# TUMFTM/global_racetrajectory_optimization

Hardware: AMD Instinct MI355X
Metric: min-curv QP solves/sec, N=2000 waypoints, batch=1024 per GPU (higher is better)
Workload: dtype f64

## Files before the change

### __graft_entry__.py

```python
import os
import subprocess
import sys
import tempfile

ROOT = os.path.dirname(os.path.abspath(__file__))
if ROOT not in sys.path:
    sys.path.insert(0, ROOT)


def build() -> None:
    env = dict(os.environ)
    env.setdefault("HIPCC", "/opt/rocm/bin/hipcc")
    fd, asm = tempfile.mkstemp(prefix="mcq_kernels_gfx950_", suffix=".s")
    os.close(fd)
    env["ASM_OUT"] = asm
    subprocess.run([os.path.join(ROOT, "global_racetrajectory_optimization_amd", "csrc", "build.sh")], check=True, env=env)
    build_variants()
    subprocess.run(["make", "-s", "-C", os.path.join(ROOT, "oracle"), "all"], check=True)
    r = subprocess.run([sys.executable, os.path.join(ROOT, "scripts", "check_csr.py"), asm], env=env)
    try:
        os.unlink(asm)
    except OSError:
        pass
    if r.returncode != 0:
        ver = subprocess.run([env["HIPCC"], "--version"], capture_output=True, text=True).stdout
        if "7.2." in ver:
            raise RuntimeError("scripts/check_csr.py found a device function that clobbers a callee-saved SGPR (see its output)")
        print("WARNING: scripts/check_csr.py reported offenders with an untested hipcc version -- not failing the build", file=sys.stderr)
    import global_racetrajectory_optimization_amd
    from global_racetrajectory_optimization_amd import engine
    lib = engine.load_library()
    for sym in engine.EXPORTED_SYMBOLS:
        assert hasattr(lib, sym), sym


VARIANTS = {"ulp": (["-DMCQ_PERTURB_ULP=1"], {}), "ipra": ([], {"IPRA": "1"}), "nocontract": (["-ffp-contract=off"], {}),
            "nof32": (["-DMCQ_IPM_F32=0"], {})}


def variant_path(name):
    return os.path.join(ROOT, "global_racetrajectory_optimization_amd", "csrc", "variants", "libmcq_%s.so" % name)


def build_variants() -> None:
    os.makedirs(os.path.dirname(variant_path("x")), exist_ok=True)
    procs = []
    for name, (flags, extra) in VARIANTS.items():
        env = dict(os.environ)
        env.setdefault("HIPCC", "/opt/rocm/bin/hipcc")
        env.pop("ASM_OUT", None)
        env.update(extra)
        env["OUT"] = variant_path(name)
        procs.append((name, subprocess.Popen([os.path.join(ROOT, "global_racetrajectory_optimization_amd", "csrc", "build.sh")] + flags, env=env)))
    for name, p in procs:
        if p.wait() != 0:
            raise RuntimeError("build of the arithmetic variant '%s' failed" % name)


def smoke() -> None:
    import numpy as np
    from global_racetrajectory_optimization_amd import engine
    from oracle import tph_ref

    g = np.load(os.path.join(ROOT, "tests", "golden", "rounded_rectangle.npz"))
    ref, nv, sc = g["reftrack"], g["normvec"], g["scaling"]
    eng = engine.Engine(0)
    al, curv, st, info = eng.solve_batch([dict(reftrack=ref, normvec=nv, scaling=sc, kappa_bound=0.12, w_veh=3.4)])
    assert st[0] == 0, "engine status %d" % st[0]
    path_cl = np.vstack((ref[:, :2], ref[0, :2]))
    _, _, A, nv_d = tph_ref.calc_splines(path_cl)
    a_ref, err_ref = tph_ref.opt_min_curv(ref, nv_d, A, 0.12, 3.4)
    d = float(np.max(np.abs(al[0] - a_ref)))
    assert d < 1e-6, "alpha differs from the oracle by %.3e m" % d
    assert abs(curv[0] - err_ref) < 1e-9
    assert float(np.max(np.abs(al[0] - g["alpha"]))) < 1e-6
    al_gi, _, st_gi, info_gi = eng.solve_batch([dict(reftrack=ref, normvec=nv, scaling=sc, kappa_bound=0.12, w_veh=3.4)], algorithm=engine.ALG_GI)
    d_gi = float(np.max(np.abs(al_gi[0] - a_ref)))
    assert st_gi[0] == 0 and info_gi[0]["gi_iters"] > 0 and d_gi < 1e-6, "Goldfarb-Idnani path: status %d, alpha differs by %.3e m" % (st_gi[0], d_gi)
    al_sp, _, st_sp, _ = eng.solve_batch([dict(reftrack=ref, normvec=nv, scaling=None, kappa_bound=1.0, w_veh=3.4)],
                                         objective=engine.OBJ_SHORTEST_PATH)
    d_sp = float(np.max(np.abs(al_sp[0] - tph_ref.opt_shortest_path(ref, nv, 3.4))))
    assert st_sp[0] == 0 and d_sp < 1e-6, "shortest path: status %d, alpha differs by %.3e m" % (st_sp[0], d_sp)
    iq = eng.iqp_batch([dict(reftrack=ref, normvectors=nv, scaling=sc)], 0.12, 3.4, 3.0, iters_min=3, curv_error_allowed=0.01)
    d_iqp = float(np.max(np.abs(iq["alpha"][0] - g["iqp_alpha"]))) if iq["alpha"][0].shape == g["iqp_alpha"].shape else float("inf")
    assert iq["status"][0] == 0 and d_iqp < 1e-6, "iqp: status %d, alpha differs by %.3e m" % (iq["status"][0], d_iqp)
    print("smoke ok: N=%d, max|alpha_gpu - alpha_oracle| = %.2e m (Goldfarb-Idnani path %.2e m in %d steps, shortest path %.2e m, iqp end state "
          "%.2e m), curv_error_max = %.6f, info = %s" % (ref.shape[0], d, d_gi, info_gi[0]["gi_iters"], d_sp, d_iqp, curv[0], info[0]))
    eng.close()


if __name__ == "__main__":
    build()
    if len(sys.argv) > 1 and sys.argv[1] == "smoke":
        smoke()
```

### global_racetrajectory_optimization_amd/csrc/mcq_kernels.hip

```cpp
#include "mcq_kernels.h"

#include <math.h>



#define MCQ_NT 256
#define MCQ_NW (MCQ_NT / 64)
typedef double d2 __attribute__((vector_size(16)));
typedef __attribute__((address_space(1))) d2 gd2;

#define SM_RED 0
#define SM_S (SM_RED + 64)
#define SPK 1920
#define SM_OVL (SM_S + SPK)
#define OVL_SIZE 7464
#define SM_KV (SM_OVL + OVL_SIZE)
#define SM_KI (SM_KV + 3 * MCQ_KMAX)
#define SM_TOTAL (SM_KI + (3 * MCQ_KMAX + 2 + 1) / 2 + 1)
static_assert(sizeof(double) * SM_TOTAL <= 80 * 1024, "two workgroups of the solver kernel per CU");

size_t mcq_solve_lds_bytes() { return sizeof(double) * SM_TOTAL; }

__shared__ double g_sm[SM_TOTAL];

#ifndef MCQ_IPM_GM_MIN
#define MCQ_IPM_GM_MIN 0.995
#endif
#ifndef MCQ_IPM_GM_C
#define MCQ_IPM_GM_C 10.0
#endif
#ifndef MCQ_TAPIA_RATIO
#define MCQ_TAPIA_RATIO 0.7
#endif
#ifndef MCQ_TAPIA_SHRINK
#define MCQ_TAPIA_SHRINK 0.7
#endif
#ifndef MCQ_WARM_ROUNDS
#define MCQ_WARM_ROUNDS 12
#endif
#define MCQ_AS_WINDOW 8

__device__ __forceinline__ int cyc1(int i, int n)
{
    i = i < 0 ? i + n : i;
    return i >= n ? i - n : i;
}

__device__ __forceinline__ int cyc(int i, int n)
{
    i %= n;
    return i < 0 ? i + n : i;
}

__device__ __forceinline__ int sdiff(int a, int b, int n)
{
    int d = cyc(a - b, n);
    return d > n / 2 ? d - n : d;
}

__device__ __forceinline__ double wave_sum(double v)
{
    for (int m = 32; m >= 1; m >>= 1) v += __shfl_xor(v, m);
    return v;
}
__device__ __forceinline__ double wave_min(double v)
{
    for (int m = 32; m >= 1; m >>= 1) v = fmin(v, __shfl_xor(v, m));
    return v;
}
__device__ __forceinline__ double wave_max(double v)
{
    for (int m = 32; m >= 1; m >>= 1) v = fmax(v, __shfl_xor(v, m));
    return v;
}

__device__ double block_reduce_(double v, int op, double* red)
{
    const int lane = threadIdx.x & 63, wv = threadIdx.x >> 6;
    v = op == 0 ? wave_sum(v) : (op == 1 ? wave_min(v) : wave_max(v));
    __syncthreads();
    if (lane == 0) red[wv] = v;
    __syncthreads();
    double r = red[0];
    for (int k = 1; k < MCQ_NW; ++k) r = op == 0 ? r + red[k] : (op == 1 ? fmin(r, red[k]) : fmax(r, red[k]));
    return r;
}

__device__ void block_reduce2_(double& a, int opa, double& b, int opb, double* red)
{
    const int lane = threadIdx.x & 63, wv = threadIdx.x >> 6;
    for (int m = 32; m >= 1; m >>= 1) {
        const double oa = __shfl_xor(a, m), ob = __shfl_xor(b, m);
        a = opa == 0 ? a + oa : (opa == 1 ? fmin(a, oa) : fmax(a, oa));
        b = opb == 0 ? b + ob : (opb == 1 ? fmin(b, ob) : fmax(b, ob));
    }
    __syncthreads();
    if (lane == 0) { red[wv] = a; red[MCQ_NW + wv] = b; }
    __syncthreads();
    double ra = red[0], rb = red[MCQ_NW];
    for (int k = 1; k < MCQ_NW; ++k) {
        ra = opa == 0 ? ra + red[k] : (opa == 1 ? fmin(ra, red[k]) : fmax(ra, red[k]));
        rb = opb == 0 ? rb + red[MCQ_NW + k] : (opb == 1 ? fmin(rb, red[MCQ_NW + k]) : fmax(rb, red[MCQ_NW + k]));
    }
    a = ra;
    b = rb;
}

struct McqSet {
    const int* n_list;
    const double* ref;
    const double* nv;
    const double* sc;
    const signed char* warm;
};
__device__ __forceinline__ McqSet mcq_set_of(const McqBatch& B)
{
    McqSet s;
    s.n_list = B.n_list; s.ref = B.ref; s.nv = B.nv; s.sc = B.sc; s.warm = B.warm;
    return s;
}

__device__ __forceinline__ McqWork mcq_work(const McqBatch& B, const McqSet& S, int pb, int& n, double& kb, double& wv)
{
    McqWork w;
    const size_t nm = (size_t)B.nmax;
    n = S.n_list ? S.n_list[pb] : B.n;
    kb = B.kappa_bound_list ? B.kappa_bound_list[pb] : B.kappa_bound;
    wv = B.w_veh_list ? B.w_veh_list[pb] : B.w_veh;
    w.ref = (const gdouble*)(S.ref + (size_t)pb * nm * 4);
    w.nv = S.nv ? (const gdouble*)(S.nv + (size_t)pb * nm * 2) : nullptr;
    w.sc = S.sc ? (const gdouble*)(S.sc + (size_t)pb * nm) : nullptr;
    w.L = (gdouble*)(B.L + (size_t)pb * nm * MCQ_LLD);
    w.vec = (gdouble*)(B.vec + (size_t)pb * nm * MCQ_NVEC);
    w.state = (gschar*)(B.state + (size_t)pb * nm);
    w.Z = (gdouble*)(B.Z + (size_t)pb * MCQ_ZLD(nm));
    w.alpha = B.alpha ? (gdouble*)(B.alpha + (size_t)pb * nm) : nullptr;
    w.curv_err = B.curv_err ? (gdouble*)(B.curv_err + pb) : nullptr;
    w.status = (gint*)(B.status + pb);
    w.info = B.info ? (ginfo*)(B.info + pb) : nullptr;
    return w;
}
__device__ __forceinline__ McqWork mcq_work(const McqBatch& B, int pb, int& n, double& kb, double& wv)
{
    return mcq_work(B, mcq_set_of(B), pb, n, kb, wv);
}

#define VEC(w, nmax, id) ((w).vec + (size_t)(id) * (size_t)(nmax))

template <int N> __device__ __forceinline__ double bcast_row16(double v)
{
    return __builtin_amdgcn_update_dpp(0.0, v, 0x150 + N, 0xf, 0xf, true);
}
#ifndef MCQ_HAVE_FNMA_BCAST_ROW16
template <int N> __device__ __forceinline__ double fnma_bcast_row16(double a, double b, double c)
{
    asm("s_nop 1\n\tv_fmac_f64_dpp %0, %1, -%2 row_newbcast:%3 row_mask:0xf bank_mask:0xf" : "+v"(c) : "v"(a), "v"(b), "n"(N));
    return c;
}
#endif

#ifndef MCQ_IPM_TOL
#define MCQ_IPM_TOL 1e-10
#endif
struct SolveCtx {
    McqDims d;
    McqWork w;
    int nm;
    int direct;
    int max_ipm_iter, max_as_iter, refine_steps;
    double zscale, fscale, wmean, nfree, kbound;
    mutable long long tk[8];
    mutable int refine_rounds, second_attempt, f32_count;
    mutable double last_step;
    mutable const gdouble* sp_sig;
    mutable const gschar* sp_mk;
    mutable const gdouble* kkt_w;
    mutable int kkt_f32;
    mutable int out_iters, out_nk;
    mutable double out_kkt;
    int chain, fix_s, fix_e;
    double psi_s, psi_e;
};
typedef __attribute__((address_space(3))) SolveCtx LCtx;
__shared__ SolveCtx g_ctx;
#define G_CTX (*(const LCtx*)&g_ctx)
#define TICK() ((long long)wall_clock64())
#include "mcq_kkt.inc"
#include "mcq_tri.inc"

#ifndef MCQ_ENTRY_BATCH
#define MCQ_ENTRY_BATCH 1
#endif
#define EB_E (MCQ_ENTRY_BATCH ? 8 : 1)
#define EB_FOR for (int eb0_ = tid; eb0_ < n; eb0_ += EB_E * MCQ_NT)
#define EB_EACH _Pragma("unroll") for (int u = 0; u < EB_E; ++u)
#define EB_INDEX                                                                                                       \
    int idx[EB_E];                                                                                                     \
    bool ok[EB_E];                                                                                                     \
    EB_EACH {                                                                                                          \
        ok[u] = eb0_ + u * MCQ_NT < n;                                                                                 \
        idx[u] = ok[u] ? eb0_ + u * MCQ_NT : eb0_;                                                                     \
    }

__device__ __noinline__ int assemble_problem(const LCtx& c, double wveh, gdouble* nv_out, gdouble* sc_out)
{
    double* red = g_sm + SM_RED;
    const int tid = threadIdx.x;
    McqWork w;
    w.ref = c.w.ref; w.nv = c.w.nv; w.sc = c.w.sc; w.L = c.w.L; w.vec = c.w.vec; w.state = c.w.state; w.Z = c.w.Z;
    w.alpha = c.w.alpha; w.curv_err = c.w.curv_err; w.status = c.w.status; w.info = c.w.info;
    const int nm = c.nm, n = c.d.n;
    gdouble* LO = VEC(w, nm, V_LO);
    gdouble* HI = VEC(w, nm, V_HI);
    gdouble* S = VEC(w, nm, V_SC);
    gdouble* XP = VEC(w, nm, V_XP);
    gdouble* YP = VEC(w, nm, V_YP);
    gdouble* CP = VEC(w, nm, V_CP);
    gdouble* KRF = VEC(w, nm, V_KREF);
    gdouble* XPP = VEC(w, nm, V_XPP);
    gdouble* YPP = VEC(w, nm, V_YPP);

    double flag_bad = 0.0, flag_inf = 0.0;
    if (n < 3) flag_bad = 1.0;
    gdouble* NX = VEC(w, nm, V_NX);
    gdouble* NY = VEC(w, nm, V_NY);
    const bool derive = w.nv == nullptr;
    const bool chain = c.chain != 0;
    if (chain && (n > MCQ_CHAIN_MAXN || derive || !(isfinite(c.psi_s) && isfinite(c.psi_e)))) flag_bad = 1.0;
    EB_FOR {
        EB_INDEX
        double rx[EB_E], ry[EB_E], rwr[EB_E], rwl[EB_E], rnx[EB_E], rny[EB_E], rs[EB_E], x1[EB_E], y1[EB_E], x2[EB_E], y2[EB_E];
        EB_EACH {
            const int i = idx[u];
            rx[u] = w.ref[4 * i]; ry[u] = w.ref[4 * i + 1]; rwr[u] = w.ref[4 * i + 2]; rwl[u] = w.ref[4 * i + 3];
            rnx[u] = derive ? 0.0 : w.nv[2 * i]; rny[u] = derive ? 1.0 : w.nv[2 * i + 1];
            rs[u] = w.sc ? w.sc[i] : 1.0;
            x1[u] = y1[u] = x2[u] = y2[u] = 0.0;
            if (derive) {
                const int i1 = i + 1 >= n ? i + 1 - n : i + 1, i2 = i1 + 1 >= n ? i1 + 1 - n : i1 + 1;
                x1[u] = w.ref[4 * i1]; y1[u] = w.ref[4 * i1 + 1]; x2[u] = w.ref[4 * i2]; y2[u] = w.ref[4 * i2 + 1];
            }
        }
        EB_EACH {
            if (!ok[u]) continue;
            const int i = idx[u];
            const double x = rx[u], y = ry[u], wr = rwr[u], wl = rwl[u];
            const double nx = rnx[u], ny = rny[u];
            double s = rs[u];
            if (chain && i >= n - 2) s = 1.0;
            if (derive) {
                const double l0 = hypot(x1[u] - x, y1[u] - y);
                const double l1 = hypot(x2[u] - x1[u], y2[u] - y1[u]);
                s = l0 / l1;
            } else {
                NX[i] = nx;
                NY[i] = ny;
            }
            if (!(isfinite(x) && isfinite(y) && isfinite(wr) && isfinite(wl) && isfinite(nx) && isfinite(ny) && isfinite(s)
                  && s > 0.0))
                flag_bad = 1.0;
            double lo = -(wl - 0.5 * wveh), hi = wr - 0.5 * wveh;
            if ((c.fix_s && i == 0) || (c.fix_e && i == n - 1)) { lo = -MCQ_FIX_HALF_WIDTH; hi = MCQ_FIX_HALF_WIDTH; }
            if (hi < lo) flag_inf = 1.0;
            LO[i] = lo;
            HI[i] = hi;
            S[i] = s;
        }
    }
    flag_bad = block_reduce_(flag_bad, 2, red);
    flag_inf = block_reduce_(flag_inf, 2, red);
    const int st = flag_bad > 0.0 ? MCQ_BAD_INPUT : (flag_inf > 0.0 ? MCQ_INFEASIBLE : MCQ_OK);
    if (tid == 0) {
        *w.status = st;
        if (w.curv_err) *w.curv_err = 0.0;
        if (w.info) {
            mcq_info z;
            z.ipm_iters = z.as_iters = z.n_active_box = z.n_active_kappa = 0;
            z.kappa_max = 0.0;
            z.kkt_res = 0.0;
            z.refine_rounds = z.second_attempt = z.f32_factorisations = z.gi_iters = 0;
            for (int q = 0; q < 8; ++q) z.ticks[q] = 0;
            *(mcq_info*)w.info = z;
        }
    }
    if (st != MCQ_OK) {
        if (w.alpha) for (int i = tid; i < n; i += MCQ_NT) w.alpha[i] = 0.0;
        return st;
    }
    __syncthreads();

    tri_prepare(c);
    gdouble* RX = VEC(w, nm, V_SK);
    gdouble* RY = VEC(w, nm, V_EDA);
    EB_FOR {
        EB_INDEX
        double sm1[EB_E], xp_[EB_E], yp_[EB_E], x0[EB_E], y0[EB_E], xm_[EB_E], ym_[EB_E];
        EB_EACH {
            const int m = idx[u], mp = cyc1(m + 1, n), mm = cyc1(m - 1, n);
            sm1[u] = S[mm];
            xp_[u] = w.ref[4 * mp]; yp_[u] = w.ref[4 * mp + 1]; x0[u] = w.ref[4 * m]; y0[u] = w.ref[4 * m + 1]; xm_[u] = w.ref[4 * mm]; ym_[u] = w.ref[4 * mm + 1];
        }
        EB_EACH if (ok[u]) {
            RX[idx[u]] = 3.0 * (sm1[u] * (xp_[u] - x0[u]) - (x0[u] - xm_[u]));
            RY[idx[u]] = 3.0 * (sm1[u] * (yp_[u] - y0[u]) - (y0[u] - ym_[u]));
        }
    }
    double hsx = 0.0, hsy = 0.0, hex = 0.0, hey = 0.0;
    if (chain) {
        hsx = MCQ_HEADING_SCALE * cos(c.psi_s + 0.5 * M_PI);
        hsy = MCQ_HEADING_SCALE * sin(c.psi_s + 0.5 * M_PI);
        hex = MCQ_HEADING_SCALE * cos(c.psi_e + 0.5 * M_PI);
        hey = MCQ_HEADING_SCALE * sin(c.psi_e + 0.5 * M_PI);
        __syncthreads();
    }
    if (chain && tid == 0) {
        RX[0] = 3.0 * ((w.ref[4] - w.ref[0]) - hsx);
        RY[0] = 3.0 * ((w.ref[5] - w.ref[1]) - hsy);
        RX[n - 1] = 3.0 * (hex - (w.ref[4 * (n - 1)] - w.ref[4 * (n - 2)]));
        RY[n - 1] = 3.0 * (hey - (w.ref[4 * (n - 1) + 1] - w.ref[4 * (n - 2) + 1]));
    }
    tri_solve_T(c, RX, XPP);
    tri_solve_T(c, RY, YPP);
    EB_FOR {
        EB_INDEX
        double a[EB_E], b[EB_E];
        EB_EACH { a[u] = XPP[idx[u]]; b[u] = YPP[idx[u]]; }
        EB_EACH if (ok[u]) { XPP[idx[u]] = a[u] * 2.0; YPP[idx[u]] = b[u] * 2.0; }
    }
    __syncthreads();

    EB_FOR {
        EB_INDEX
        double si[EB_E], xn_[EB_E], yn_[EB_E], x0[EB_E], y0[EB_E], ax[EB_E], axn[EB_E], ay[EB_E], ayn[EB_E];
        EB_EACH {
            const int i = idx[u], ip = cyc(i + 1, n);
            si[u] = S[i];
            xn_[u] = w.ref[4 * ip]; yn_[u] = w.ref[4 * ip + 1]; x0[u] = w.ref[4 * i]; y0[u] = w.ref[4 * i + 1];
            ax[u] = XPP[i]; axn[u] = XPP[ip]; ay[u] = YPP[i]; ayn[u] = YPP[ip];
        }
        EB_EACH {
            if (!ok[u]) continue;
            const int i = idx[u];
            const double s2 = si[u] * si[u];
            const double xp = (xn_[u] - x0[u]) - (ax[u] + 0.5 * s2 * axn[u]) / 3.0;
            const double yp = (yn_[u] - y0[u]) - (ay[u] + 0.5 * s2 * ayn[u]) / 3.0;
            const double den = pow(xp * xp + yp * yp, 1.5);
            const double cp = den != 0.0 ? 1.0 / den : 0.0;
            XP[i] = xp;
            YP[i] = yp;
            CP[i] = cp;
            KRF[i] = cp * (xp * ay[u] - yp * ax[u]);
            if (derive) {
                const double nrm = sqrt(xp * xp + yp * yp);
                NX[i] = yp / nrm;
                NY[i] = -xp / nrm;
            }
            if (nv_out) {
                nv_out[2 * i] = NX[i];
                nv_out[2 * i + 1] = NY[i];
            }
            if (sc_out) sc_out[i] = si[u];
        }
    }
    if (chain) {
        __syncthreads();
        if (tid == 0) {
            const int i = n - 1;
            const double den = pow(hex * hex + hey * hey, 1.5);
            const double cp = den != 0.0 ? 1.0 / den : 0.0;
            XP[i] = hex;
            YP[i] = hey;
            CP[i] = cp;
            KRF[i] = cp * (hex * YPP[i] - hey * XPP[i]);
        }
    }
    __syncthreads();
    return MCQ_OK;
}

__device__ __forceinline__ void ctx_set_problem(const McqBatch& B, const McqSet& S, int pb, int& n, double& kb, double& wveh)
{
    const McqWork w = mcq_work(B, S, pb, n, kb, wveh);
    __syncthreads();
    if (threadIdx.x == 0) {
        g_ctx.w = w;
        g_ctx.nm = B.nmax;
        g_ctx.d = mcq_dims(n);
        const mcq_ends* e = B.ends ? B.ends + pb : nullptr;
        g_ctx.chain = (e && !e->closed) ? 1 : 0;
        g_ctx.fix_s = g_ctx.chain && e->fix_s;
        g_ctx.fix_e = g_ctx.chain && e->fix_e;
        g_ctx.psi_s = g_ctx.chain ? e->psi_s : 0.0;
        g_ctx.psi_e = g_ctx.chain ? e->psi_e : 0.0;
    }
    __syncthreads();
}

__device__ __forceinline__ void ctx_set_problem(const McqBatch& B, int pb, int& n, double& kb, double& wveh)
{
    ctx_set_problem(B, mcq_set_of(B), pb, n, kb, wveh);
}

__device__ __forceinline__ void ctx_set_solve(const McqBatch& B, double kbound)
{
    if (threadIdx.x == 0) {
        for (int q = 0; q < 8; ++q) g_ctx.tk[q] = 0;
        g_ctx.last_step = 0.0;
        g_ctx.refine_rounds = g_ctx.second_attempt = g_ctx.f32_count = 0;
        g_ctx.direct = B.objective == MCQ_OBJ_SHORTEST_PATH;
        g_ctx.max_ipm_iter = B.max_ipm_iter;
        g_ctx.max_as_iter = B.max_as_iter;
        g_ctx.refine_steps = B.refine_steps;
        g_ctx.kbound = kbound;
        g_ctx.kkt_w = nullptr;
        g_ctx.kkt_f32 = 0;
        g_ctx.sp_sig = nullptr;
        g_ctx.sp_mk = nullptr;
        g_ctx.out_iters = g_ctx.out_nk = 0;
        g_ctx.out_kkt = 0.0;
    }
    __syncthreads();
}

__global__ void __launch_bounds__(MCQ_NT) mcq_assemble_kernel(McqBatch B)
{
    int n;
    double kb, wveh;
    ctx_set_problem(B, blockIdx.x, n, kb, wveh);
    const size_t nm = (size_t)B.nmax;
    (void)assemble_problem(G_CTX, wveh, B.nv_out ? (gdouble*)(B.nv_out + (size_t)blockIdx.x * nm * 2) : nullptr,
                           B.sc_out ? (gdouble*)(B.sc_out + (size_t)blockIdx.x * nm) : nullptr);
}

__global__ void __launch_bounds__(MCQ_NT) mcq_assemble_sp_kernel(McqBatch B)
{
    __shared__ double red[64];
    const int tid = threadIdx.x;
    int n;
    double kb, wveh;
    const McqWork w = mcq_work(B, blockIdx.x, n, kb, wveh);
    const int nm = B.nmax;
    gdouble* LO = VEC(w, nm, V_LO);
    gdouble* HI = VEC(w, nm, V_HI);
    gdouble* NX = VEC(w, nm, V_NX);
    gdouble* NY = VEC(w, nm, V_NY);
    gdouble* F = VEC(w, nm, V_F);
    gdouble* KRF = VEC(w, nm, V_KREF);

    double flag_bad = n < 3 ? 1.0 : 0.0;
    for (int i = tid; i < n; i += MCQ_NT) {
        const double x = w.ref[4 * i], y = w.ref[4 * i + 1], wr = w.ref[4 * i + 2], wl = w.ref[4 * i + 3];
        const double nx = w.nv[2 * i], ny = w.nv[2 * i + 1];
        if (!(isfinite(x) && isfinite(y) && isfinite(wr) && isfinite(wl) && isfinite(nx) && isfinite(ny))) flag_bad = 1.0;
        NX[i] = nx;
        NY[i] = ny;
        LO[i] = -fmax(wl - 0.5 * wveh, 0.001);
        HI[i] = fmax(wr - 0.5 * wveh, 0.001);
        KRF[i] = 0.0;
    }
    flag_bad = block_reduce_(flag_bad, 2, red);
    const int st = flag_bad > 0.0 ? MCQ_BAD_INPUT : MCQ_OK;
    if (tid == 0) {
        *w.status = st;
        if (w.curv_err) *w.curv_err = 0.0;
        if (w.info) {
            mcq_info z;
            z.ipm_iters = z.as_iters = z.n_active_box = z.n_active_kappa = 0;
            z.kappa_max = 0.0;
            z.kkt_res = 0.0;
            z.refine_rounds = z.second_attempt = z.f32_factorisations = z.gi_iters = 0;
            for (int q = 0; q < 8; ++q) z.ticks[q] = 0;
            *(mcq_info*)w.info = z;
        }
    }
    if (st != MCQ_OK) {
        if (w.alpha) for (int i = tid; i < n; i += MCQ_NT) w.alpha[i] = 0.0;
        return;
    }

    gdouble* HD = VEC(w, nm, V_XP);
    gdouble* HU = VEC(w, nm, V_YP);
    for (int i = tid; i < n; i += MCQ_NT) {
        const int ip = i + 1 == n ? 0 : i + 1, im = i == 0 ? n - 1 : i - 1;
        HD[i] = 4.0 * (w.nv[2 * i] * w.nv[2 * i] + w.nv[2 * i + 1] * w.nv[2 * i + 1]);
        HU[i] = -2.0 * (w.nv[2 * i] * w.nv[2 * ip] + w.nv[2 * i + 1] * w.nv[2 * ip + 1]);
        const double px = w.ref[4 * i], py = w.ref[4 * i + 1];
        F[i] = 2.0 * (w.nv[2 * i] * ((px - w.ref[4 * im]) - (w.ref[4 * ip] - px))
                      + w.nv[2 * i + 1] * ((py - w.ref[4 * im + 1]) - (w.ref[4 * ip + 1] - py)));
    }
}


__device__ __noinline__ int factor(const LCtx& c, const gdouble* sig, const gschar* mk, gdouble* fv, bool f32)
{
    if (c.direct) return factor_sp(c, sig, mk);
    c.kkt_f32 = f32 ? 1 : 0;
    if (threadIdx.x == 0) c.f32_count += f32 ? 1 : 0;
    return f32 ? factor_kkt<true>(c, sig, mk, c.kkt_w, fv) : factor_kkt<false>(c, sig, mk, c.kkt_w, fv);
}

__device__ __noinline__ void solve(const LCtx& c, gdouble* v, bool fwd_done)
{
    if (c.direct) { (void)sp_solve(c, v, v); return; }
    if (c.kkt_f32) solve_kkt<true>(c, v, fwd_done);
    else solve_kkt<false>(c, v, fwd_done);
}

__device__ __forceinline__ void apply_Et(const LCtx& c, const gdouble* src, gdouble* dst) { tri_apply_Et(c, src, dst); }

__device__ __noinline__ void gradient(const LCtx& c, const gdouble* x, const gdouble* extra, gdouble* tmp, gdouble* g)
{
    const int n = c.d.n;
    const long long t0 = TICK();
    __syncthreads();
    if (c.direct) {
        const gdouble* HD = VEC(c.w, c.nm, V_SPD);
        const gdouble* HU = VEC(c.w, c.nm, V_SPU);
        const gdouble* F = VEC(c.w, c.nm, V_F);
        for (int i = threadIdx.x; i < n; i += MCQ_NT) {
            const int im = i > 0 ? i - 1 : n - 1, ip = i + 1 < n ? i + 1 : 0;
            g[i] = F[i] + HU[im] * x[im] + HD[i] * x[i] + HU[i] * x[ip];
        }
        __syncthreads();
        if (threadIdx.x == 0) c.tk[2] += TICK() - t0;
        return;
    }
    tri_apply_E(c, x, VEC(c.w, c.nm, V_KREF), MCQ_F_SCALE, tmp);
    if (extra) {
        for (int i = threadIdx.x; i < n; i += MCQ_NT) tmp[i] += extra[i];
        __syncthreads();
    }
    tri_apply_Et(c, tmp, g);
    if (threadIdx.x == 0) c.tk[2] += TICK() - t0;
}

__device__ __forceinline__ int timed_factor(const LCtx& c, const gdouble* sig, const gschar* mk, gdouble* fv = nullptr, bool f32 = false)
{
    const long long t0 = TICK();
    const int r = factor(c, sig, mk, fv, f32);
    if (threadIdx.x == 0) c.tk[0] += TICK() - t0;
    return r;
}
__device__ __forceinline__ void timed_solve(const LCtx& c, gdouble* v, bool fwd_done = false)
{
    const long long t0 = TICK();
    solve(c, v, fwd_done);
    if (threadIdx.x == 0) c.tk[1] += TICK() - t0;
}


__device__ __noinline__ int ipm(const LCtx& c, bool with_kappa)
{
    const int tid = threadIdx.x, n = c.d.n, nm = c.nm;
    double* red = g_sm + SM_RED;
    const gdouble* LO = VEC(c.w, nm, V_LO);
    const gdouble* HI = VEC(c.w, nm, V_HI);
    const gdouble* KR = VEC(c.w, nm, V_KREF);
    gdouble* X = VEC(c.w, nm, V_X);
    gdouble* G = VEC(c.w, nm, V_G);
    gdouble* ZL = VEC(c.w, nm, V_ZL);
    gdouble* ZU = VEC(c.w, nm, V_ZU);
    gdouble* SIG = VEC(c.w, nm, V_SIG);
    gdouble* RHS = VEC(c.w, nm, V_RHS);
    gdouble* DXA = VEC(c.w, nm, V_DXA);
    gdouble* T0 = VEC(c.w, nm, V_T0);
    gdouble* T1 = VEC(c.w, nm, V_T1);
    gdouble* T2 = VEC(c.w, nm, V_T2);
    gdouble* TL = VEC(c.w, nm, V_TL);
    gdouble* TU = VEC(c.w, nm, V_TU);
    gdouble* YL = VEC(c.w, nm, V_YL);
    gdouble* YU = VEC(c.w, nm, V_YU);
    gdouble* SK = VEC(c.w, nm, V_SK);
    gdouble* EDA = VEC(c.w, nm, V_EDA);
    gdouble* Q = VEC(c.w, nm, V_Q);
    gschar* ST = c.w.state;
    const double kb = c.kbound, zscale = c.zscale;
    const double IPM_TOL = 1e-10;
    c.out_iters = 0;

    for (int i = tid; i < n; i += MCQ_NT) {
        const bool fixed = !(HI[i] - LO[i] > 1e-12);
        ST[i] = fixed ? 2 : 0;
        X[i] = 0.5 * (LO[i] + HI[i]);
        ZL[i] = fixed ? 0.0 : zscale;
        ZU[i] = ZL[i];
    }
    __syncthreads();
    if (with_kappa) {
        tri_apply_E(c, X, KR, 1.0, T0);
        const double mu0 = 0.5 * zscale * c.wmean;
        for (int i = tid; i < n; i += MCQ_NT) {
            const double r = T0[i];
            const double tl = fmax(kb + r, 0.1 * kb), tu = fmax(kb - r, 0.1 * kb);
            TL[i] = tl; TU[i] = tu;
            YL[i] = mu0 / tl; YU[i] = mu0 / tu;
        }
        __syncthreads();
    }
    const double npairs = 2.0 * c.nfree + (with_kappa ? 2.0 * n : 0.0);
    const gschar* const no_mask = nullptr;
    const bool any_fixed = c.nfree < (double)n;
    (void)no_mask;
    if (!(npairs > 0.0)) return MCQ_OK;

    bool g_exact = true;
    double mu_first = 0.0, rdm_best = 1e300;
    for (int it = 1; it <= c.max_ipm_iter; ++it) {
        if (with_kappa) {
            for (int i = tid; i < n; i += MCQ_NT) Q[i] = YU[i] - YL[i];
            gradient(c, X, Q, T0, T1);
            gradient(c, X, nullptr, T0, G);
            tri_apply_E(c, X, KR, 1.0, T0);
        }
        double mu, rdm, rhom;
        for (;;) {
            mu = 0.0; rdm = 0.0; rhom = 0.0;
            for (int i = tid; i < n; i += MCQ_NT) {
                if (with_kappa) {
                    mu += TL[i] * YL[i] + TU[i] * YU[i];
                    rhom = fmax(rhom, fmax(fabs(TL[i] - (kb + T0[i])), fabs(TU[i] - (kb - T0[i]))));
                    SK[i] = YL[i] / TL[i] + YU[i] / TU[i];
                }
                if (ST[i] != 0) continue;
                const double sl = X[i] - LO[i], su = HI[i] - X[i];
                mu += sl * ZL[i] + su * ZU[i];
                const double gg = with_kappa ? T1[i] : G[i];
                rdm = fmax(rdm, fabs(gg - ZL[i] + ZU[i]));
                SIG[i] = ZL[i] / sl + ZU[i] / su;
            }
            mu = block_reduce_(mu, 0, red) / npairs;
            rdm = block_reduce_(rdm, 2, red);
            rhom = block_reduce_(rhom, 2, red);
            const bool conv = mu < IPM_TOL * zscale * c.wmean && rdm < IPM_TOL * zscale && rhom <= 1e-9 * kb;
            if (with_kappa && it > 1 && mu < 1e-6 * mu_first && rdm > 10.0 * rdm_best) return MCQ_OK;
            rdm_best = fmin(rdm_best, rdm);
#ifdef IPM_TRACE
            if (tid == 0) printf("ipm%d it %d mu %.3e rdm %.3e rhom %.3e step %.3e\n", (int)with_kappa, it, mu / (zscale * c.wmean), rdm / zscale, rhom / kb, c.last_step);
#endif
            if (conv && (with_kappa || g_exact)) return MCQ_OK;
            if (!conv) break;
            gradient(c, X, nullptr, T0, G);
            g_exact = true;
        }
        c.out_iters = it;
        if (it == 1) mu_first = mu;

        int fs;
        if (with_kappa) {
            for (int i = tid; i < n; i += MCQ_NT) EDA[i] = 1.0 + SK[i];
            __syncthreads();
            c.kkt_w = EDA;
            fs = timed_factor(c, SIG, any_fixed ? ST : nullptr);
            c.kkt_w = nullptr;
            if (fs == MCQ_NOT_PD && mu < 1e-6 * mu_first) return MCQ_OK;
        } else {
            fs = timed_factor(c, SIG, any_fixed ? ST : nullptr);
        }
        if (fs != 0) return fs;

        if (with_kappa) {
            for (int i = tid; i < n; i += MCQ_NT) {
                const double rl = TL[i] - (kb + T0[i]), ru = TU[i] - (kb - T0[i]);
                Q[i] = YL[i] * rl / TL[i] - YU[i] * ru / TU[i];
            }
            __syncthreads();
            apply_Et(c, Q, T2);
            __syncthreads();
            for (int i = tid; i < n; i += MCQ_NT) RHS[i] = ST[i] == 0 ? -G[i] + T2[i] : 0.0;
        } else {
            for (int i = tid; i < n; i += MCQ_NT) RHS[i] = ST[i] == 0 ? -G[i] : 0.0;
        }
        timed_solve(c, RHS);
        if (with_kappa) {
            tri_apply_E(c, RHS, nullptr, 0.0, EDA);
        }
        double ap = 1.0, ad = 1.0;
        for (int i = tid; i < n; i += MCQ_NT) {
            if (with_kappa) {
                const double rl = TL[i] - (kb + T0[i]), ru = TU[i] - (kb - T0[i]);
                const double dtl = EDA[i] - rl, dtu = -EDA[i] - ru;
                const double dyl = -YL[i] - YL[i] * dtl / TL[i], dyu = -YU[i] - YU[i] * dtu / TU[i];
                if (dtl < 0.0) ap = fmin(ap, -TL[i] / dtl);
                if (dtu < 0.0) ap = fmin(ap, -TU[i] / dtu);
                if (dyl < 0.0) ad = fmin(ad, -YL[i] / dyl);
                if (dyu < 0.0) ad = fmin(ad, -YU[i] / dyu);
            }
            if (ST[i] != 0) { DXA[i] = 0.0; continue; }
            const double dx = RHS[i];
            DXA[i] = dx;
            const double sl = X[i] - LO[i], su = HI[i] - X[i];
            const double dzl = -ZL[i] - ZL[i] * dx / sl, dzu = -ZU[i] + ZU[i] * dx / su;
            if (dx < 0.0) ap = fmin(ap, -sl / dx);
            if (dx > 0.0) ap = fmin(ap, su / dx);
            if (dzl < 0.0) ad = fmin(ad, -ZL[i] / dzl);
            if (dzu < 0.0) ad = fmin(ad, -ZU[i] / dzu);
        }
        ap = block_reduce_(ap, 1, red);
        ad = block_reduce_(ad, 1, red);
        double mua = 0.0;
        for (int i = tid; i < n; i += MCQ_NT) {
            if (with_kappa) {
                const double rl = TL[i] - (kb + T0[i]), ru = TU[i] - (kb - T0[i]);
                const double dtl = EDA[i] - rl, dtu = -EDA[i] - ru;
                const double dyl = -YL[i] - YL[i] * dtl / TL[i], dyu = -YU[i] - YU[i] * dtu / TU[i];
                mua += (TL[i] + ap * dtl) * (YL[i] + ad * dyl) + (TU[i] + ap * dtu) * (YU[i] + ad * dyu);
            }
            if (ST[i] != 0) continue;
            const double dx = DXA[i];
            const double sl = X[i] - LO[i], su = HI[i] - X[i];
            const double dzl = -ZL[i] - ZL[i] * dx / sl, dzu = -ZU[i] + ZU[i] * dx / su;
            mua += (sl + ap * dx) * (ZL[i] + ad * dzl) + (su - ap * dx) * (ZU[i] + ad * dzu);
        }
        mua = block_reduce_(mua, 0, red) / npairs;
        const double ratio = mua / mu;
        const double smu = ratio * ratio * ratio * mu;

        if (with_kappa) {
            for (int i = tid; i < n; i += MCQ_NT) {
                const double rl = TL[i] - (kb + T0[i]), ru = TU[i] - (kb - T0[i]);
                const double dtl = EDA[i] - rl, dtu = -EDA[i] - ru;
                const double dyl = -YL[i] - YL[i] * dtl / TL[i], dyu = -YU[i] - YU[i] * dtu / TU[i];
                Q[i] = (smu - dtl * dyl + YL[i] * rl) / TL[i] - (smu - dtu * dyu + YU[i] * ru) / TU[i];
            }
            __syncthreads();
            apply_Et(c, Q, T2);
            __syncthreads();
        }
        for (int i = tid; i < n; i += MCQ_NT) {
            if (ST[i] != 0) { RHS[i] = 0.0; continue; }
            const double dx = DXA[i];
            const double sl = X[i] - LO[i], su = HI[i] - X[i];
            const double dzl = -ZL[i] - ZL[i] * dx / sl, dzu = -ZU[i] + ZU[i] * dx / su;
            RHS[i] = -G[i] + (smu - dx * dzl) / sl - (smu + dx * dzu) / su + (with_kappa ? T2[i] : 0.0);
        }
        timed_solve(c, RHS);
        if (with_kappa) {
            tri_apply_E(c, RHS, nullptr, 0.0, Q);
        }
        double amax = 1.0 / 0.995;
        for (int i = tid; i < n; i += MCQ_NT) {
            if (with_kappa) {
                const double rl = TL[i] - (kb + T0[i]), ru = TU[i] - (kb - T0[i]);
                const double dtla = EDA[i] - rl, dtua = -EDA[i] - ru;
                const double dyla = -YL[i] - YL[i] * dtla / TL[i], dyua = -YU[i] - YU[i] * dtua / TU[i];
                const double dtl = Q[i] - rl, dtu = -Q[i] - ru;
                const double dyl = (-TL[i] * YL[i] + smu - dtla * dyla - YL[i] * dtl) / TL[i];
                const double dyu = (-TU[i] * YU[i] + smu - dtua * dyua - YU[i] * dtu) / TU[i];
                EDA[i] = dyl;
                SK[i] = dyu;
                if (dtl < 0.0) amax = fmin(amax, -TL[i] / dtl);
                if (dtu < 0.0) amax = fmin(amax, -TU[i] / dtu);
                if (dyl < 0.0) amax = fmin(amax, -YL[i] / dyl);
                if (dyu < 0.0) amax = fmin(amax, -YU[i] / dyu);
            }
            if (ST[i] != 0) continue;
            const double dx = RHS[i], da = DXA[i];
            const double sl = X[i] - LO[i], su = HI[i] - X[i];
            const double dzla = -ZL[i] - ZL[i] * da / sl, dzua = -ZU[i] + ZU[i] * da / su;
            const double dzl = (-sl * ZL[i] + smu - da * dzla - ZL[i] * dx) / sl;
            const double dzu = (-su * ZU[i] + smu + da * dzua + ZU[i] * dx) / su;
            T1[i] = dzl;
            T2[i] = dzu;
            if (dx < 0.0) amax = fmin(amax, -sl / dx);
            if (dx > 0.0) amax = fmin(amax, su / dx);
            if (dzl < 0.0) amax = fmin(amax, -ZL[i] / dzl);
            if (dzu < 0.0) amax = fmin(amax, -ZU[i] / dzu);
        }
        amax = block_reduce_(amax, 1, red);
        const double a = fmin(1.0, 0.995 * amax);
        c.last_step = a;
        for (int i = tid; i < n; i += MCQ_NT) {
            if (with_kappa) {
                const double rl = TL[i] - (kb + T0[i]), ru = TU[i] - (kb - T0[i]);
                TL[i] += a * (Q[i] - rl);
                TU[i] += a * (-Q[i] - ru);
                YL[i] += a * EDA[i];
                YU[i] += a * SK[i];
            }
            if (ST[i] != 0) continue;
            if (!with_kappa) {
                const double dxa = DXA[i], dx = RHS[i];
                const double sl = X[i] - LO[i], su = HI[i] - X[i];
                const double dzla = -ZL[i] - ZL[i] * dxa / sl, dzua = -ZU[i] + ZU[i] * dxa / su;
                const double rc = -G[i] + (smu - dxa * dzla) / sl - (smu + dxa * dzua) / su;
                G[i] += a * (rc - SIG[i] * dx);
            }
            {
                const double sl = X[i] - LO[i], su = HI[i] - X[i];
                const double rsl = (sl + a * RHS[i]) * ZL[i], rzl = (ZL[i] + a * T1[i]) * sl;
                const double rsu = (su - a * RHS[i]) * ZU[i], rzu = (ZU[i] + a * T2[i]) * su;
                const bool al = rsl < MCQ_TAPIA_RATIO * rzl && sl + a * RHS[i] < MCQ_TAPIA_SHRINK * sl, au = rsu < MCQ_TAPIA_RATIO * rzu && su - a * RHS[i] < MCQ_TAPIA_SHRINK * su;
                VEC(c.w, nm, V_T3)[i] = al ? -1.0 : (au ? 1.0 : 0.0);
            }
            X[i] += a * RHS[i];
            ZL[i] += a * T1[i];
            ZU[i] += a * T2[i];
        }
        g_exact = false;
        __syncthreads();
    }
    return with_kappa ? MCQ_KAPPA_INFEASIBLE : MCQ_ITER_CAP;
}

#define IPB_E 8
#define IPB_H 4
#ifndef MCQ_IPB_RESIDENT
#define MCQ_IPB_RESIDENT 1
#endif
#ifndef MCQ_IPB_DEFER
#define MCQ_IPB_DEFER MCQ_IPB_RESIDENT
#endif
#ifndef MCQ_IPB_NOCOPY
#define MCQ_IPB_NOCOPY MCQ_IPB_RESIDENT
#endif
#if MCQ_IPB_DEFER && !MCQ_IPB_RESIDENT
#error "MCQ_IPB_DEFER needs MCQ_IPB_RESIDENT"
#endif
#ifndef MCQ_IPB_FOLD_P1
#define MCQ_IPB_FOLD_P1 1
#endif
__device__ __noinline__ int ipm_box(const LCtx& c, double tol, bool resume)
{
#define IPB_SETUP                                                                                                      \
    const int tid = threadIdx.x, n = c.d.n, nm = c.nm;                                                                 \
    double* red = g_sm + SM_RED;                                                                                       \
    const gdouble* LO = VEC(c.w, nm, V_LO);                                                                            \
    const gdouble* HI = VEC(c.w, nm, V_HI);                                                                            \
    gdouble* X = VEC(c.w, nm, V_X);                                                                                    \
    gdouble* G = VEC(c.w, nm, V_G);                                                                                    \
    gdouble* ZL = VEC(c.w, nm, V_ZL);                                                                                  \
    gdouble* ZU = VEC(c.w, nm, V_ZU);                                                                                  \
    gdouble* SIG = VEC(c.w, nm, V_SIG);                                                                                \
    gdouble* RHS = VEC(c.w, nm, V_RHS);                                                                                \
    gdouble* DXA = VEC(c.w, nm, V_DXA);                                                                                \
    gschar* ST = c.w.state;                                                                                            \
    gdouble* IND = VEC(c.w, nm, V_T3);                                                                                 \
    (void)IND; (void)red; (void)LO; (void)HI; (void)X; (void)G; (void)ZL; (void)ZU; (void)SIG; (void)RHS; (void)DXA; (void)ST;    \
    int idx[IPB_E];                                                                                                    \
    bool ok[IPB_E];                                                                                                    \
    _Pragma("unroll") for (int u = 0; u < IPB_E; ++u) {                                                                \
        ok[u] = tid + u * MCQ_NT < n;                                                                                  \
        idx[u] = ok[u] ? tid + u * MCQ_NT : 0;           \
    }
#define IPB_HALF(h)                                                                                                    \
    int idx[IPB_H];                                                                                                    \
    bool ok[IPB_H];                                                                                                    \
    _Pragma("unroll") for (int u = 0; u < IPB_H; ++u) {                                                                \
        ok[u] = tid + ((h) * IPB_H + u) * MCQ_NT < n;                                                                  \
        idx[u] = ok[u] ? tid + ((h) * IPB_H + u) * MCQ_NT : 0;                                                         \
    }
#define IPB_PTRS                                                                                                       \
    const int tid = threadIdx.x, n = c.d.n, nm = c.nm;                                                                 \
    double* red = g_sm + SM_RED;                                                                                       \
    const gdouble* LO = VEC(c.w, nm, V_LO);                                                                            \
    const gdouble* HI = VEC(c.w, nm, V_HI);                                                                            \
    gdouble* X = VEC(c.w, nm, V_X);                                                                                    \
    gdouble* G = VEC(c.w, nm, V_G);                                                                                    \
    gdouble* ZL = VEC(c.w, nm, V_ZL);                                                                                  \
    gdouble* ZU = VEC(c.w, nm, V_ZU);                                                                                  \
    gdouble* SIG = VEC(c.w, nm, V_SIG);                                                                                \
    gdouble* RHS = VEC(c.w, nm, V_RHS);                                                                                \
    gdouble* DXA = VEC(c.w, nm, V_DXA);                                                                                \
    gschar* ST = c.w.state;                                                                                            \
    gdouble* IND = VEC(c.w, nm, V_T3);                                                                                 \
    (void)IND; (void)red; (void)LO; (void)HI; (void)X; (void)G; (void)ZL; (void)ZU; (void)SIG; (void)RHS; (void)DXA; (void)ST;
#if MCQ_IPB_NOCOPY
#define IPB_CORR DXA
#define IPB_PRED RHS
#else
#define IPB_CORR RHS
#define IPB_PRED DXA
#endif
    const double zscale = c.zscale;
    const double IPM_TOL = tol;
    c.out_iters = 0;
    {
    IPB_SETUP
#if MCQ_ENTRY_BATCH
    double lo[IPB_E], hi[IPB_E];
#pragma unroll
    for (int u = 0; u < IPB_E; ++u) { lo[u] = LO[idx[u]]; hi[u] = HI[idx[u]]; }
#define IPB_LO(u, i) lo[u]
#define IPB_HI(u, i) hi[u]
#else
#define IPB_LO(u, i) LO[i]
#define IPB_HI(u, i) HI[i]
#endif
#pragma unroll
    for (int u = 0; u < IPB_E; ++u) {
        if (!ok[u]) continue;
        const int i = idx[u];
        const bool fixed = !(IPB_HI(u, i) - IPB_LO(u, i) > 1e-12);
        ST[i] = fixed ? 2 : 0;
        if (!resume) {
            X[i] = 0.5 * (IPB_LO(u, i) + IPB_HI(u, i));
            ZL[i] = fixed ? 0.0 : zscale;
            ZU[i] = ZL[i];
        }
    }
#undef IPB_LO
#undef IPB_HI
    }
    __syncthreads();
    if (resume) gradient(c, VEC(c.w, c.nm, V_X), nullptr, VEC(c.w, c.nm, V_T0), VEC(c.w, c.nm, V_G));
    const double npairs = 2.0 * c.nfree;
    const bool any_fixed = c.nfree < (double)c.d.n;
    if (!(npairs > 0.0)) return MCQ_OK;
#if MCQ_IPB_RESIDENT
    double rx[IPB_E], rl[IPB_E], ru[IPB_E], rg[IPB_E];
    {
        IPB_SETUP
#pragma unroll
        for (int u = 0; u < IPB_E; ++u) { const int i = idx[u]; rx[u] = X[i]; rl[u] = ZL[i]; ru[u] = ZU[i]; rg[u] = G[i]; }
    }
#define IPB_RELOAD_G { _Pragma("unroll") for (int u = 0; u < IPB_E; ++u) rg[u] = G[tid + u * MCQ_NT < n ? tid + u * MCQ_NT : 0]; }
#else
#define IPB_RELOAD_G
#endif
#if MCQ_IPB_DEFER
#define IPB_STORE_X { _Pragma("unroll") for (int u = 0; u < IPB_E; ++u) if (tid + u * MCQ_NT < n) X[tid + u * MCQ_NT] = rx[u]; }
#define IPB_RETURN(v) { rc = (v); goto ipb_flush; }
    unsigned tapia = 0;
    int rc;
#else
#define IPB_STORE_X
#define IPB_RETURN(v) return (v);
#endif

    bool g_exact = true;
    double mu_prev = 1e300;
    int stalled = 0;
#ifndef MCQ_IPM_F32
#define MCQ_IPM_F32 1
#endif
#ifndef MCQ_IPM_F32_RD
#define MCQ_IPM_F32_RD 1e-5
#endif
    bool f32 = MCQ_IPM_F32 && !resume;
#ifndef MCQ_IPM_TRUST_FP64_CARRY
#define MCQ_IPM_TRUST_FP64_CARRY 1
#endif
    bool g_f32 = false;
#if MCQ_IPB_FOLD_P1
    bool folded = false;
    double mu_fold = 0.0, rdm_fold = 0.0;
#endif
    for (int it = 1; it <= c.max_ipm_iter; ++it) {
        double mu;
        for (;;) {
            IPB_PTRS
            double rdm = 0.0;
            mu = 0.0;
#if MCQ_IPB_FOLD_P1
            if (folded) { mu = mu_fold; rdm = rdm_fold; folded = false; }
            else
#endif
            {
#pragma unroll
            for (int h = 0; h < IPB_E / IPB_H; ++h) {
                IPB_HALF(h)
                double x[IPB_H], lo[IPB_H], hi[IPB_H], zl[IPB_H], zu[IPB_H], g[IPB_H];
                int st[IPB_H];
#pragma unroll
                for (int u = 0; u < IPB_H; ++u) {
                    const int i = idx[u];
#if MCQ_IPB_RESIDENT
                    st[u] = ST[i]; lo[u] = LO[i]; hi[u] = HI[i];
                    x[u] = rx[h * IPB_H + u]; zl[u] = rl[h * IPB_H + u]; zu[u] = ru[h * IPB_H + u]; g[u] = rg[h * IPB_H + u];
#else
                    st[u] = ST[i]; x[u] = X[i]; lo[u] = LO[i]; hi[u] = HI[i]; zl[u] = ZL[i]; zu[u] = ZU[i]; g[u] = G[i];
#endif
                }
#pragma unroll
                for (int u = 0; u < IPB_H; ++u) {
                    if (!ok[u]) continue;
                    const int i = idx[u];
                    if (st[u] != 0) { RHS[i] = 0.0; continue; }
                    const double sl = x[u] - lo[u], su = hi[u] - x[u];
                    mu += sl * zl[u] + su * zu[u];
                    rdm = fmax(rdm, fabs(g[u] - zl[u] + zu[u]));
                    SIG[i] = zl[u] / sl + zu[u] / su;
                    RHS[i] = -g[u];
                }
            }
            block_reduce2_(mu, 0, rdm, 2, red);
            mu /= npairs;
            }
            const bool conv = mu < IPM_TOL * zscale * c.wmean && rdm < IPM_TOL * zscale;
#ifdef IPM_TRACE
            if (threadIdx.x == 0) printf("ipmb it %d mu %.3e rdm %.3e exact %d resume %d [%a %a]\n", it, mu / (zscale * c.wmean), rdm / zscale, (int)g_exact, (int)resume, mu, rdm);
#endif
            if (f32 && it > 1 && rdm < MCQ_IPM_F32_RD * zscale) {
                f32 = false;
                if (!g_exact) {
                    IPB_STORE_X
                    gradient(c, X, nullptr, VEC(c.w, nm, V_T0), G);
                    IPB_RELOAD_G
                    g_exact = true;
                    g_f32 = false;
                    continue;
                }
            }
            if (conv && (g_exact || (MCQ_IPM_TRUST_FP64_CARRY && !resume && !g_f32))) IPB_RETURN(MCQ_OK)
            if (!conv) break;
            IPB_STORE_X
            gradient(c, X, nullptr, VEC(c.w, nm, V_T0), G);
            IPB_RELOAD_G
            g_exact = true;
            g_f32 = false;
        }
        c.out_iters = it;
        if (resume) {
            stalled = mu > 0.9 * mu_prev ? stalled + 1 : 0;
            mu_prev = mu;
            if (stalled >= 3) IPB_RETURN(MCQ_OK)
        }

        const int fs = timed_factor(c, VEC(c.w, c.nm, V_SIG), any_fixed ? c.w.state : nullptr,
                                    VEC(c.w, c.nm, V_RHS), f32);
        if (fs != 0) IPB_RETURN((resume && fs == MCQ_NOT_PD) ? MCQ_OK : fs)
        timed_solve(c, VEC(c.w, c.nm, V_RHS), true);

        double smu;
        {
            IPB_SETUP
            double dxa[IPB_E], sl[IPB_E], su[IPB_E], zl[IPB_E], zu[IPB_E], g[IPB_E];
            bool act[IPB_E];
#pragma unroll
            for (int u = 0; u < IPB_E; ++u) {
                const int i = idx[u];
                act[u] = ok[u] && ST[i] == 0;
#if MCQ_IPB_RESIDENT
                const double x = rx[u];
                dxa[u] = RHS[i]; sl[u] = x - LO[i]; su[u] = HI[i] - x; zl[u] = rl[u]; zu[u] = ru[u]; g[u] = rg[u];
#else
                const double x = X[i];
                dxa[u] = RHS[i]; sl[u] = x - LO[i]; su[u] = HI[i] - x; zl[u] = ZL[i]; zu[u] = ZU[i]; g[u] = G[i];
#endif
            }
            double ap = 1.0, ad = 1.0;
#pragma unroll
            for (int u = 0; u < IPB_E; ++u) {
                if (!ok[u]) continue;
#if MCQ_IPB_NOCOPY
                if (!act[u]) continue;
                const double dx = dxa[u];
#else
                if (!act[u]) { DXA[idx[u]] = 0.0; continue; }
                const double dx = dxa[u];
                DXA[idx[u]] = dx;
#endif
                const double dzla = -zl[u] - zl[u] * dx / sl[u];
                const double dzua = -zu[u] + zu[u] * dx / su[u];
                if (dx < 0.0) ap = fmin(ap, -sl[u] / dx);
                if (dx > 0.0) ap = fmin(ap, su[u] / dx);
                if (dzla < 0.0) ad = fmin(ad, -zl[u] / dzla);
                if (dzua < 0.0) ad = fmin(ad, -zu[u] / dzua);
            }
            block_reduce2_(ap, 1, ad, 1, red);
            double mua = 0.0;
#pragma unroll
            for (int u = 0; u < IPB_E; ++u) {
                if (!act[u]) continue;
                const double dzla = -zl[u] - zl[u] * dxa[u] / sl[u];
                const double dzua = -zu[u] + zu[u] * dxa[u] / su[u];
                mua += (sl[u] + ap * dxa[u]) * (zl[u] + ad * dzla) + (su[u] - ap * dxa[u]) * (zu[u] + ad * dzua);
            }
            mua = block_reduce_(mua, 0, red) / npairs;
            const double ratio = mua / mu;
            smu = ratio * ratio * ratio * mu;
#pragma unroll
            for (int u = 0; u < IPB_E; ++u) {
                if (!ok[u]) continue;
                const double dzla = -zl[u] - zl[u] * dxa[u] / sl[u];
                const double dzua = -zu[u] + zu[u] * dxa[u] / su[u];
                IPB_CORR[idx[u]] = act[u] ? -g[u] + (smu - dxa[u] * dzla) / sl[u] - (smu + dxa[u] * dzua) / su[u] : 0.0;
            }
        }
        timed_solve(c, VEC(c.w, c.nm, MCQ_IPB_NOCOPY ? V_DXA : V_RHS));

        {
            IPB_SETUP
#ifdef MCQ_IPM_FIXED_STEP
            const double gm = 0.995;
#else
            const double gm = fmin(fmax(MCQ_IPM_GM_MIN, 1.0 - MCQ_IPM_GM_C * mu / (zscale * c.wmean)), 1.0 - 1e-9);
#endif
            double amax = 1.0 / gm;
            double dx[IPB_E], da[IPB_E], x[IPB_E], lo[IPB_E], hi[IPB_E], zl[IPB_E], zu[IPB_E], g[IPB_E], sg[IPB_E];
            bool act[IPB_E];
#pragma unroll
            for (int u = 0; u < IPB_E; ++u) {
                const int i = idx[u];
                act[u] = ok[u] && ST[i] == 0;
                dx[u] = IPB_CORR[i]; da[u] = IPB_PRED[i]; lo[u] = LO[i]; hi[u] = HI[i]; sg[u] = SIG[i];
#if MCQ_IPB_RESIDENT
                x[u] = rx[u]; zl[u] = rl[u]; zu[u] = ru[u]; g[u] = rg[u];
#else
                x[u] = X[i]; zl[u] = ZL[i]; zu[u] = ZU[i]; g[u] = G[i];
#endif
            }
#define IPB_STEP3(u)                                                                                                          \
                const double sl = x[u] - lo[u], su = hi[u] - x[u];                                                              \
                const double dzla = -zl[u] - zl[u] * da[u] / sl, dzua = -zu[u] + zu[u] * da[u] / su;                             \
                const double dzl = (-sl * zl[u] + smu - da[u] * dzla - zl[u] * dx[u]) / sl;                                     \
                const double dzu = (-su * zu[u] + smu + da[u] * dzua + zu[u] * dx[u]) / su;
#pragma unroll
            for (int u = 0; u < IPB_E; ++u) {
                if (!act[u]) continue;
                IPB_STEP3(u)
                if (dx[u] < 0.0) amax = fmin(amax, -sl / dx[u]);
                if (dx[u] > 0.0) amax = fmin(amax, su / dx[u]);
                if (dzl < 0.0) amax = fmin(amax, -zl[u] / dzl);
                if (dzu < 0.0) amax = fmin(amax, -zu[u] / dzu);
            }
            amax = block_reduce_(amax, 1, red);
            const double a = fmin(1.0, gm * amax);
            c.last_step = a;
#if MCQ_IPB_DEFER
            unsigned t3[IPB_E];
#pragma unroll
            for (int u = 0; u < IPB_E; ++u) t3[u] = 0;
#endif
#if MCQ_IPB_FOLD_P1
            double mu_n = 0.0, rdm_n = 0.0;
#endif
#pragma unroll
            for (int u = 0; u < IPB_E; ++u) {
#if MCQ_IPB_FOLD_P1
                if (ok[u] && !act[u]) RHS[idx[u]] = 0.0;
#endif
                if (!act[u]) continue;
                const int i = idx[u];
                IPB_STEP3(u)
                const double rc = -g[u] + (smu - da[u] * dzla) / sl - (smu + da[u] * dzua) / su;
                const double hdx = rc - sg[u] * dx[u];
                const double gn = g[u] + a * hdx, xn = x[u] + a * dx[u], zln = zl[u] + a * dzl, zun = zu[u] + a * dzu;
#if MCQ_IPB_RESIDENT
                rg[u] = gn; rx[u] = xn; rl[u] = zln; ru[u] = zun;
#endif
#if !MCQ_IPB_DEFER
                G[i] = gn;
                X[i] = xn;
                ZL[i] = zln;
                ZU[i] = zun;
#endif
                const double rsl = (sl + a * dx[u]) * zl[u], rzl = (zl[u] + a * dzl) * sl;
                const double rsu = (su - a * dx[u]) * zu[u], rzu = (zu[u] + a * dzu) * su;
                const bool al = rsl < MCQ_TAPIA_RATIO * rzl && sl + a * dx[u] < MCQ_TAPIA_SHRINK * sl, au = rsu < MCQ_TAPIA_RATIO * rzu && su - a * dx[u] < MCQ_TAPIA_SHRINK * su;
#if MCQ_IPB_DEFER
                t3[u] = al ? 1u : (au ? 3u : 2u);
                (void)i;
#else
                IND[i] = al ? -1.0 : (au ? 1.0 : 0.0);
#endif
#if MCQ_IPB_FOLD_P1
                {
                    const double sl = xn - lo[u], su = hi[u] - xn;
                    mu_n += sl * zln + su * zun;
                    rdm_n = fmax(rdm_n, fabs(gn - zln + zun));
                    SIG[idx[u]] = zln / sl + zun / su;
                    RHS[idx[u]] = -gn;
                }
#endif
            }
#if MCQ_IPB_FOLD_P1
            block_reduce2_(mu_n, 0, rdm_n, 2, red);
            mu_fold = mu_n / npairs;
            rdm_fold = rdm_n;
            folded = true;
#endif
#if MCQ_IPB_DEFER
            tapia = 0;
#pragma unroll
            for (int u = 0; u < IPB_E; ++u) tapia |= t3[u] << (2 * u);
#endif
#undef IPB_STEP3
        }
        g_exact = false;
        g_f32 |= f32;
#if !MCQ_IPB_FOLD_P1
        __syncthreads();
#endif
    }
#if MCQ_IPB_DEFER
    rc = MCQ_ITER_CAP;
ipb_flush:
    {
        IPB_SETUP
#pragma unroll
        for (int u = 0; u < IPB_E; ++u) {
            if (!ok[u]) continue;
            const int i = idx[u];
            X[i] = rx[u]; ZL[i] = rl[u]; ZU[i] = ru[u]; G[i] = rg[u];
            const unsigned t = (tapia >> (2 * u)) & 3u;
            if (t != 0) IND[i] = (double)((int)t - 2);
        }
    }
    __syncthreads();
    return rc;
#else
    return MCQ_ITER_CAP;
#endif
#undef IPB_SETUP
#undef IPB_RELOAD_G
#undef IPB_STORE_X
#undef IPB_RETURN
#undef IPB_CORR
#undef IPB_PRED
}

struct KappaMem {
    double* kmu;
    double* krh;
    double* mul;
    int* ki;
    int* piv;
    gdouble* sg;
    int cap, ld;
    bool in_lds;
};
__device__ __forceinline__ KappaMem kappa_mem_lds(const LCtx& c)
{
    KappaMem k;
    k.kmu = g_sm + SM_KV;
    k.krh = g_sm + SM_KV + MCQ_KMAX;
    k.mul = g_sm + SM_KV + 2 * MCQ_KMAX;
    k.ki = (int*)(g_sm + SM_KI);
    k.piv = (int*)(g_sm + SM_KI) + 1 + 2 * MCQ_KMAX;
    k.sg = c.w.Z + c.nm;
    k.cap = MCQ_KMAX;
    k.ld = MCQ_KMAX;
    k.in_lds = true;
    return k;
}
__device__ __forceinline__ KappaMem kappa_mem_slot(double* slot)
{
    KappaMem k;
    k.sg = (gdouble*)slot;
    double* v = slot + (size_t)MCQ_KBIG * MCQ_KBIG;
    k.kmu = v;
    k.krh = v + MCQ_KBIG;
    k.mul = v + 2 * MCQ_KBIG;
    k.ki = (int*)(v + 3 * MCQ_KBIG);
    k.piv = k.ki + 2 + 2 * MCQ_KBIG;
    k.cap = MCQ_KBIG;
    k.ld = MCQ_KBIG;
    k.in_lds = false;
    return k;
}

template <typename PA>
__device__ __forceinline__ void kappa_lu_eliminate(PA A, int lda, int nk, double* mul, int* piv)
{
    const int tid = threadIdx.x;
    double* red = g_sm + SM_RED;
    for (int cidx = 0; cidx < nk; ++cidx) {
        double best = -1.0;
        int brow = cidx;
        for (int r = cidx + tid; r < nk; r += MCQ_NT) {
            const double v = fabs(A[(size_t)r * lda + cidx]);
            if (v > best) { best = v; brow = r; }
        }
        const double bmax = block_reduce_(best, 2, red);
        double cand = (best == bmax && best >= 0.0) ? (double)brow : 1e300;
        cand = block_reduce_(cand, 1, red);
        const int pr = cand < 1e299 ? (int)cand : cidx;
        if (tid == 0) piv[cidx] = pr;
        if (pr != cidx)
            for (int cc = tid; cc < nk; cc += MCQ_NT) {
                const double t = A[(size_t)cidx * lda + cc];
                A[(size_t)cidx * lda + cc] = A[(size_t)pr * lda + cc];
                A[(size_t)pr * lda + cc] = t;
            }
        __syncthreads();
        const double pv = A[(size_t)cidx * lda + cidx];
        for (int r = cidx + 1 + tid; r < nk; r += MCQ_NT) mul[r] = pv != 0.0 ? A[(size_t)r * lda + cidx] / pv : 0.0;
        __syncthreads();
        const int rem = nk - cidx - 1;
        for (int e = tid; e < rem * rem; e += MCQ_NT) {
            const int r = cidx + 1 + e / rem, cc = cidx + 1 + e % rem;
            A[(size_t)r * lda + cc] -= mul[r] * A[(size_t)cidx * lda + cc];
        }
        __syncthreads();
        for (int r = cidx + 1 + tid; r < nk; r += MCQ_NT) A[(size_t)r * lda + cidx] = mul[r];
        __syncthreads();
    }
}

__device__ void kappa_lu_factor(const KappaMem& K, int nk)
{
    const int tid = threadIdx.x;
    __syncthreads();
    if (K.in_lds && nk * nk <= OVL_SIZE) {
        double* A = g_sm + SM_OVL;
        for (int e = tid; e < nk * nk; e += MCQ_NT) A[e] = K.sg[(size_t)(e / nk) * K.ld + (e % nk)];
        __syncthreads();
        kappa_lu_eliminate(A, nk, nk, K.mul, K.piv);
        for (int e = tid; e < nk * nk; e += MCQ_NT) K.sg[(size_t)(e / nk) * K.ld + (e % nk)] = A[e];
    } else {
        kappa_lu_eliminate(K.sg, K.ld, nk, K.mul, K.piv);
    }
    __syncthreads();
}

template <typename PA>
__device__ __forceinline__ void kappa_lu_substitute(PA A, int lda, int nk, double* KMU, const int* piv)
{
    const int tid = threadIdx.x;
    if (tid == 0)
        for (int cidx = 0; cidx < nk; ++cidx) {
            const int pr = piv[cidx];
            if (pr != cidx) { const double t = KMU[cidx]; KMU[cidx] = KMU[pr]; KMU[pr] = t; }
        }
    __syncthreads();
    for (int cidx = 0; cidx < nk; ++cidx) {
        const double yc = KMU[cidx];
        __syncthreads();
        for (int r = cidx + 1 + tid; r < nk; r += MCQ_NT) KMU[r] -= A[(size_t)r * lda + cidx] * yc;
        __syncthreads();
    }
    for (int cidx = nk - 1; cidx >= 0; --cidx) {
        if (tid == 0) { const double pv = A[(size_t)cidx * lda + cidx]; KMU[cidx] = pv != 0.0 ? KMU[cidx] / pv : 0.0; }
        __syncthreads();
        const double xc = KMU[cidx];
        for (int r = tid; r < cidx; r += MCQ_NT) KMU[r] -= A[(size_t)r * lda + cidx] * xc;
        __syncthreads();
    }
}

__device__ void kappa_lu_solve(const KappaMem& K, int nk)
{
    const int tid = threadIdx.x;
    __syncthreads();
    for (int q = tid; q < nk; q += MCQ_NT) K.kmu[q] = K.krh[q];
    if (K.in_lds && nk * nk <= OVL_SIZE) {
        double* A = g_sm + SM_OVL;
        for (int e = tid; e < nk * nk; e += MCQ_NT) A[e] = K.sg[(size_t)(e / nk) * K.ld + (e % nk)];
        __syncthreads();
        kappa_lu_substitute((const double*)A, nk, nk, K.kmu, K.piv);
    } else {
        __syncthreads();
        kappa_lu_substitute((const gdouble*)K.sg, K.ld, nk, K.kmu, K.piv);
    }
}

__device__ void kappa_apply(const LCtx& c, const KappaMem& K, int nk, gdouble* Q, gdouble* v)
{
    const int tid = threadIdx.x, n = c.d.n;
    const double* KMU = K.kmu;
    const int* KI = K.ki;
    const gschar* ST = c.w.state;
    for (int i = tid; i < n; i += MCQ_NT) Q[i] = 0.0;
    __syncthreads();
    for (int q = tid; q < nk; q += MCQ_NT) Q[KI[1 + q]] = KMU[q];
    __syncthreads();
    apply_Et(c, Q, v);
    __syncthreads();
    for (int i = tid; i < n; i += MCQ_NT) if (ST[i] != 0) v[i] = 0.0;
    __syncthreads();
    timed_solve(c, v);
}

__device__ __noinline__ int active_set(const LCtx& c, bool with_kappa, bool tapia, int cap, int identify, const KappaMem K)
{
    const int tid = threadIdx.x, n = c.d.n, nm = c.nm;
    double* red = g_sm + SM_RED;
    double* KMU = K.kmu;
    double* KRH = K.krh;
    int* KI = K.ki;
    const int kcap = K.cap;
    const gdouble* LO = VEC(c.w, nm, V_LO);
    const gdouble* HI = VEC(c.w, nm, V_HI);
    const gdouble* KR = VEC(c.w, nm, V_KREF);
    gdouble* X = VEC(c.w, nm, V_X);
    gdouble* G = VEC(c.w, nm, V_G);
    gdouble* ZL = VEC(c.w, nm, V_ZL);
    gdouble* ZU = VEC(c.w, nm, V_ZU);
    gdouble* RHS = VEC(c.w, nm, V_RHS);
    gdouble* T0 = VEC(c.w, nm, V_T0);
    gdouble* T1 = VEC(c.w, nm, V_T1);
    gdouble* T2 = VEC(c.w, nm, V_T2);
    gdouble* T3 = VEC(c.w, nm, V_T3);
    gdouble* Q = VEC(c.w, nm, V_Q);
    gdouble* KF = VEC(c.w, nm, V_SK);
    gdouble* PV = VEC(c.w, nm, V_DXA);
    gschar* ST = c.w.state;
    const double zscale = c.zscale, fscale = c.fscale, kb = c.kbound;
    const int win = MCQ_AS_WINDOW < (n - 1) / 2 ? MCQ_AS_WINDOW : (n - 1) / 2;
    c.out_iters = 0;
    c.out_kkt = 0.0;
    c.out_nk = 0;

    EB_FOR {
        EB_INDEX
        signed char st0[EB_E];
        double lo[EB_E], hi[EB_E], x[EB_E], zl[EB_E], zu[EB_E], t3[EB_E];
        if (identify == 1) {
            EB_EACH {
                const int i = idx[u];
                st0[u] = ST[i]; lo[u] = LO[i]; hi[u] = HI[i]; x[u] = X[i]; zl[u] = ZL[i]; zu[u] = ZU[i];
                t3[u] = tapia ? VEC(c.w, nm, V_T3)[i] : 0.0;
            }
        }
        EB_EACH {
            if (!ok[u]) continue;
            const int i = idx[u];
            if (identify == 1 && st0[u] == 0) {
                const double wdt = hi[u] - lo[u];
                const double sl = x[u] - lo[u], su = hi[u] - x[u];
                signed char st = 0;
                if (sl * zscale < zl[u] * wdt) st = -1;
                else if (su * zscale < zu[u] * wdt) st = 1;
                if (tapia && st == 0) st = (signed char)t3[u];
                ST[i] = st;
            }
            double kf = 0.0;
            if (with_kappa && identify == 2) kf = KF[i];
            else if (with_kappa) {
                const gdouble* TL = VEC(c.w, nm, V_TL);
                const gdouble* TU = VEC(c.w, nm, V_TU);
                const gdouble* YL = VEC(c.w, nm, V_YL);
                const gdouble* YU = VEC(c.w, nm, V_YU);
                const double mu0 = 0.5 * zscale * c.wmean;
                if (TL[i] * mu0 < YL[i] * kb * kb) kf = -1.0;
                else if (TU[i] * mu0 < YU[i] * kb * kb) kf = 1.0;
            }
            KF[i] = kf;
        }
    }
    __syncthreads();
    const double TOLX = 1e-10;
    const double toly = 1e-10 * (fscale > 0.0 ? fscale : 1.0);
    const double tolk = 1e-10 * kb;
    int best = 2 * n + 1, pcnt = 3;
    for (int it = 1; it <= cap; ++it) {
        c.out_iters = it;
        if (tid == 0) {
            int nk = 0;
            if (with_kappa)
                for (int i = 0; i < n; ++i)
                    if (KF[i] != 0.0 && nk < kcap + 1) {
                        if (nk < kcap) { KI[1 + nk] = i; KI[1 + kcap + nk] = KF[i] > 0.0 ? 1 : -1; }
                        ++nk;
                    }
            KI[0] = nk;
        }
        __syncthreads();
        const int nk = KI[0];
        if (nk > kcap) return MCQ_KAPPA_ACTIVE;
        c.out_nk = nk;

        EB_FOR {
            EB_INDEX
            signed char st[EB_E];
            double lo[EB_E], hi[EB_E];
            EB_EACH { const int i = idx[u]; st[u] = ST[i]; lo[u] = LO[i]; hi[u] = HI[i]; }
            EB_EACH if (ok[u]) T1[idx[u]] = st[u] == 0 ? 0.0 : (st[u] < 0 ? lo[u] : (st[u] == 1 ? hi[u] : 0.5 * (lo[u] + hi[u])));
        }
        gradient(c, T1, nullptr, T0, T2);
        EB_FOR {
            EB_INDEX
            signed char st[EB_E];
            double t1[EB_E], t2[EB_E];
            EB_EACH { const int i = idx[u]; st[u] = ST[i]; t1[u] = T1[i]; t2[u] = T2[i]; }
            EB_EACH if (ok[u]) RHS[idx[u]] = st[u] == 0 ? -t2[u] : t1[u];
        }
        const int fs = timed_factor(c, nullptr, ST, RHS);
        if (fs != 0) return fs;
        timed_solve(c, RHS, true);
        if (nk > 0) {
            gdouble* Zs = c.w.Z;
            gdouble* SG = K.sg;
            for (int q = 0; q < nk; ++q) {
                const int k = KI[1 + q];
                for (int i = tid; i < n; i += MCQ_NT) T2[i] = i == k ? 1.0 : 0.0;
                apply_Et(c, T2, Zs);
                for (int i = tid; i < n; i += MCQ_NT) if (ST[i] != 0) Zs[i] = 0.0;
                __syncthreads();
                timed_solve(c, Zs);
                tri_apply_E(c, Zs, nullptr, 0.0, T0);
                for (int q2 = tid; q2 < nk; q2 += MCQ_NT) SG[(size_t)q2 * K.ld + q] = T0[KI[1 + q2]];
                __syncthreads();
            }
            tri_apply_E(c, RHS, KR, 1.0, T0);
            for (int q = tid; q < nk; q += MCQ_NT) KRH[q] = T0[KI[1 + q]] - KI[1 + kcap + q] * kb;
            kappa_lu_factor(K, nk);
            kappa_lu_solve(K, nk);
            kappa_apply(c, K, nk, Q, Zs);
            for (int i = tid; i < n; i += MCQ_NT) RHS[i] -= Zs[i];
            __syncthreads();
        }
        EB_FOR {
            EB_INDEX
            signed char st[EB_E];
            double t1[EB_E], rh[EB_E];
            EB_EACH { const int i = idx[u]; st[u] = ST[i]; t1[u] = T1[i]; rh[u] = RHS[i]; }
            EB_EACH if (ok[u]) X[idx[u]] = st[u] == 0 ? rh[u] : t1[u];
        }
        gradient(c, X, nk > 0 ? Q : nullptr, T0, G);
        if (with_kappa) tri_apply_E(c, X, KR, 1.0, T2);
        double nv = 0.0, imax = -1.0, kk = 0.0;
        EB_FOR {
            EB_INDEX
            signed char sta[EB_E];
            double x[EB_E], lo[EB_E], hi[EB_E], g[EB_E];
            EB_EACH { const int i = idx[u]; sta[u] = ST[i]; x[u] = X[i]; lo[u] = LO[i]; hi[u] = HI[i]; g[u] = G[i]; }
            EB_EACH {
                if (!ok[u]) continue;
                const int i = idx[u];
                const signed char st = sta[u];
                int v = 0;
                double pv = 0.0;
                if (st == 0) {
                    if (x[u] < lo[u] - TOLX) { v = -1; pv = lo[u] - x[u]; }
                    else if (x[u] > hi[u] + TOLX) { v = 1; pv = x[u] - hi[u]; }
                    kk = fmax(kk, fabs(g[u]));
                } else if (st == -1) { if (g[u] < -toly) v = 2; }
                else if (st == 1) { if (g[u] > toly) v = 2; }
                PV[i] = pv;
                int vk = 0;
                if (with_kappa) {
                    const double kf = KF[i];
                    if (kf == 0.0) {
                        if (T2[i] > kb + tolk) vk = 1;
                        else if (T2[i] < -kb - tolk) vk = -1;
                    } else if (kf * Q[i] < -toly) vk = 2;
                }
                T3[i] = (double)(v + 8 * vk);
                if (v != 0) { nv += 1.0; imax = fmax(imax, (double)i); }
                if (vk != 0) { nv += 1.0; imax = fmax(imax, (double)(n + i)); }
            }
        }
        nv = block_reduce_(nv, 0, red);
        imax = block_reduce_(imax, 2, red);
        c.out_kkt = block_reduce_(kk, 2, red);
        const int nvi = (int)nv;
        if (nvi == 0) {
            for (int r = 0; r < c.refine_steps; ++r) {
                EB_FOR {
                    EB_INDEX
                    signed char st[EB_E];
                    double g[EB_E];
                    EB_EACH { const int i = idx[u]; st[u] = ST[i]; g[u] = G[i]; }
                    EB_EACH if (ok[u]) RHS[idx[u]] = st[u] == 0 ? -g[u] : 0.0;
                }
                timed_solve(c, RHS);
                if (nk > 0) {
                    gdouble* Zs = c.w.Z;
                    tri_apply_E(c, RHS, nullptr, 0.0, T0);
                    for (int q = tid; q < nk; q += MCQ_NT) {
                        const int k = KI[1 + q];
                        KRH[q] = T0[k] + T2[k] - KI[1 + kcap + q] * kb;
                    }
                    kappa_lu_solve(K, nk);
                    for (int q = tid; q < nk; q += MCQ_NT) KRH[q] = KMU[q];
                    __syncthreads();
                    kappa_apply(c, K, nk, T1, Zs);
                    for (int i = tid; i < n; i += MCQ_NT) RHS[i] -= Zs[i];
                    __syncthreads();
                    for (int q = tid; q < nk; q += MCQ_NT) Q[KI[1 + q]] += KRH[q];
                    __syncthreads();
                }
                double dm = 0.0;
                EB_FOR {
                    EB_INDEX
                    signed char st[EB_E];
                    double x[EB_E], rh[EB_E];
                    EB_EACH { const int i = idx[u]; st[u] = ST[i]; x[u] = X[i]; rh[u] = RHS[i]; }
                    EB_EACH if (ok[u] && st[u] == 0) { X[idx[u]] = x[u] + rh[u]; dm = fmax(dm, fabs(rh[u])); }
                }
                dm = block_reduce_(dm, 2, red);
                gradient(c, X, nk > 0 ? Q : nullptr, T0, G);
                if (nk > 0) tri_apply_E(c, X, KR, 1.0, T2);
                c.refine_rounds = r + 1;
                if (!(dm > 1e-8)) break;
            }
            double k2 = 0.0;
            EB_FOR {
                EB_INDEX
                signed char st[EB_E];
                double g[EB_E];
                EB_EACH { const int i = idx[u]; st[u] = ST[i]; g[u] = G[i]; }
                EB_EACH if (ok[u] && st[u] == 0) k2 = fmax(k2, fabs(g[u]));
            }
            c.out_kkt = block_reduce_(k2, 2, red);
            return MCQ_OK;
        }
        bool full;
        if (nvi < best) { best = nvi; pcnt = 3; full = true; }
        else if (pcnt > 0) { --pcnt; full = true; }
        else if (with_kappa) return MCQ_ITER_CAP;
        else full = false;
        for (int i = tid; i < n; i += MCQ_NT) {
            const int code = (int)T3[i];
            int vk = (code + 20) / 8 - 2;
            int v = code - 8 * vk;
            if (v > 2) { v -= 8; vk += 1; }
            if (v != 0 && (full || i == (int)imax)) {
                bool take = true;
                if (full && v != 2) {
                    const double me = PV[i];
                    for (int o = 1; o <= win && take; ++o)
                        if (PV[cyc1(i - o, n)] >= me || PV[cyc1(i + o, n)] > me) take = false;
                }
                if (take) ST[i] = v == 2 ? 0 : (signed char)v;
            }
            if (vk != 0 && (full || n + i == (int)imax)) KF[i] = vk == 2 ? 0.0 : (double)vk;
        }
        __syncthreads();
    }
    return MCQ_ITER_CAP;
}

__device__ int claim_slot(int* flags, int nslots, bool wait)
{
    int* sh = (int*)(g_sm + SM_RED);
    __syncthreads();
    if (threadIdx.x == 0) {
        int got = -1;
        for (;;) {
            const int s0 = (int)(blockIdx.x % (unsigned)nslots);
            for (int k = 0; k < nslots && got < 0; ++k) {
                const int s = s0 + k < nslots ? s0 + k : s0 + k - nslots;
                if (atomicCAS(flags + s, 0, 1) == 0) got = s;
            }
            if (got >= 0 || !wait) break;
            for (int r = 0; r < 64; ++r) __builtin_amdgcn_s_sleep(127);
        }
        sh[0] = got;
    }
    __syncthreads();
    const int slot = sh[0];
    __syncthreads();
    return slot;
}
__device__ void release_slot(int* flags, int slot)
{
    __syncthreads();
    if (threadIdx.x == 0) { __threadfence(); atomicExch(flags + slot, 0); }
}

#ifdef MCQ_OUTLINE_PROLOGUE
#define MCQ_FN_PROLOGUE __device__ __noinline__
#else
#define MCQ_FN_PROLOGUE __device__ __forceinline__
#endif
MCQ_FN_PROLOGUE void problem_scales(const LCtx& c)
{
    const int tid = threadIdx.x, n = c.d.n, nm = c.nm;
    double* red = g_sm + SM_RED;
    const gdouble* LO = VEC(c.w, nm, V_LO);
    const gdouble* HI = VEC(c.w, nm, V_HI);
    const gdouble* F = VEC(c.w, nm, V_F);
    gdouble* X = VEC(c.w, nm, V_X);
    gdouble* G = VEC(c.w, nm, V_G);
    gschar* ST = c.w.state;
    double wsum = 0.0, nfree_d = 0.0, fmaxl = 0.0;
    EB_FOR {
        EB_INDEX
        double lo[EB_E], hi[EB_E], f[EB_E];
        EB_EACH { const int i = idx[u]; lo[u] = LO[i]; hi[u] = HI[i]; f[u] = F[i]; }
        EB_EACH {
            if (!ok[u]) continue;
            const int i = idx[u];
            const double wdt = hi[u] - lo[u];
            const bool fixed = !(wdt > 1e-12);
            ST[i] = fixed ? 2 : 0;
            X[i] = 0.5 * (lo[u] + hi[u]);
            if (!fixed) { wsum += wdt; nfree_d += 1.0; }
            fmaxl = fmax(fmaxl, fabs(f[u]));
        }
    }
    wsum = block_reduce_(wsum, 0, red);
    const double nfree_s = block_reduce_(nfree_d, 0, red), fscale_s = block_reduce_(fmaxl, 2, red);
    gradient(c, X, nullptr, VEC(c.w, nm, V_T0), G);
    double gm = 0.0;
    EB_FOR {
        EB_INDEX
        signed char st[EB_E];
        double g[EB_E];
        EB_EACH { const int i = idx[u]; st[u] = ST[i]; g[u] = G[i]; }
        EB_EACH if (ok[u] && st[u] == 0) gm = fmax(gm, fabs(g[u]));
    }
    double zscale_s = block_reduce_(gm, 2, red);
    if (!(zscale_s > 0.0)) zscale_s = fscale_s > 0.0 ? fscale_s : 1.0;
    if (tid == 0) {
        g_ctx.nfree = nfree_s;
        g_ctx.fscale = fscale_s;
        g_ctx.wmean = nfree_s > 0.0 ? wsum / nfree_s : 1.0;
        g_ctx.zscale = zscale_s;
    }
    __syncthreads();
}

struct McqOutcome {
    int status, ipm_iters, as_iters, nact_kappa, gi_iters;
    double kkt, km;
    bool dd_valid;
    long long t_kernel0, c_kernel0, t_epi0;
};
MCQ_FN_PROLOGUE void write_outputs(const LCtx& c, const McqOutcome& r)
{
    const int tid = threadIdx.x, n = c.d.n, nm = c.nm;
    double* red = g_sm + SM_RED;
    const gdouble* X = VEC(c.w, nm, V_X);
    gdouble* T0 = VEC(c.w, nm, V_T0);
    gdouble* T1 = VEC(c.w, nm, V_T1);
    gdouble* T2 = VEC(c.w, nm, V_T2);
    gdouble* T3 = VEC(c.w, nm, V_T3);
    gdouble* Q = VEC(c.w, nm, V_Q);
    const gschar* ST = c.w.state;
    double nact = 0.0;
    EB_FOR {
        EB_INDEX
        signed char st[EB_E];
        double x[EB_E];
        EB_EACH { const int i = idx[u]; st[u] = ST[i]; x[u] = X[i]; }
        EB_EACH {
            if (!ok[u]) continue;
            c.w.alpha[idx[u]] = x[u];
            if (st[u] == -1 || st[u] == 1) nact += 1.0;
        }
    }
    nact = block_reduce_(nact, 0, red);
    const gdouble* XP = VEC(c.w, nm, V_XP);
    const gdouble* YP = VEC(c.w, nm, V_YP);
    const gdouble* XPP = VEC(c.w, nm, V_XPP);
    const gdouble* YPP = VEC(c.w, nm, V_YPP);
    if (!c.direct) {
        EB_FOR {
            EB_INDEX
            double nx[EB_E], ny[EB_E], x[EB_E];
            EB_EACH { const int i = idx[u]; nx[u] = VEC(c.w, nm, V_NX)[i]; ny[u] = VEC(c.w, nm, V_NY)[i]; x[u] = X[i]; }
            EB_EACH if (ok[u]) { T1[idx[u]] = nx[u] * x[u]; T2[idx[u]] = ny[u] * x[u]; }
        }
        __syncthreads();
        if (r.dd_valid) {
            const gdouble* D1 = VEC(c.w, nm, V_TL);
            const gdouble* D2 = VEC(c.w, nm, V_TU);
            EB_FOR {
                EB_INDEX
                double d1[EB_E], d2[EB_E];
                EB_EACH { d1[u] = D1[idx[u]]; d2[u] = D2[idx[u]]; }
                EB_EACH if (ok[u]) { T0[idx[u]] = d1[u]; T3[idx[u]] = d2[u]; }
            }
        } else {
            tri_apply_E(c, X, nullptr, 0.0, Q, T0, T3);
        }
        __syncthreads();
    }
    double em = 0.0;
    for (int i = tid; i < (c.direct ? 0 : n); i += MCQ_NT) {
        const int ip = cyc(i + 1, n);
        const double s = VEC(c.w, nm, V_SC)[i];
        const double s2 = s * s;
        double xpt = XP[i] + (T1[ip] - T1[i]) - (T0[i] + 0.5 * s2 * T0[ip]) / 3.0;
        double ypt = YP[i] + (T2[ip] - T2[i]) - (T3[i] + 0.5 * s2 * T3[ip]) / 3.0;
        if (c.chain && i == n - 1) { xpt = XP[i]; ypt = YP[i]; }
        const double xpp = XPP[i] + T0[i], ypp = YPP[i] + T3[i];
        const double xp = XP[i], yp = YP[i];
        const double k0 = (xp * ypp - yp * xpp) / pow(xp * xp + yp * yp, 1.5);
        const double k1 = (xpt * ypp - ypt * xpp) / pow(xpt * xpt + ypt * ypt, 1.5);
        em = fmax(em, fabs(k1 - k0));
    }
    em = block_reduce_(em, 2, red);
    if (tid == 0) {
        *c.w.curv_err = em;
        *c.w.status = r.status;
        if (c.w.info) {
            mcq_info o;
            o.ipm_iters = r.ipm_iters;
            o.as_iters = r.as_iters;
            o.n_active_box = (int)nact;
            o.n_active_kappa = r.nact_kappa;
            o.kappa_max = r.km;
            o.kkt_res = c.fscale > 0.0 ? r.kkt / c.fscale : r.kkt;
            o.refine_rounds = c.refine_rounds;
            o.second_attempt = c.second_attempt;
            o.f32_factorisations = c.f32_count;
            o.gi_iters = r.gi_iters;
            c.tk[3] = TICK() - r.t_kernel0;
            c.tk[7] = TICK() - r.t_epi0;
            c.tk[6] = (long long)clock64() - r.c_kernel0;
            for (int q = 0; q < 8; ++q) o.ticks[q] = c.tk[q];
            *(mcq_info*)c.w.info = o;
        }
    }
}

#include "mcq_gi.inc"

__device__ __forceinline__ void solve_body(const McqBatch& B, const McqSet& IN, const int pb)
{
    const int tid = threadIdx.x;
    int n;
    double kbound, wveh;
    if (B.poison_lds) {
        for (int q = tid; q < SM_TOTAL; q += MCQ_NT) g_sm[q] = __longlong_as_double(-1LL);
        __syncthreads();
    }
    const long long t_kernel0 = TICK();
    const long long c_kernel0 = (long long)clock64();
    ctx_set_problem(B, IN, pb, n, kbound, wveh);
    const LCtx& c = G_CTX;
    ctx_set_solve(B, kbound);
    if (B.objective == MCQ_OBJ_SHORTEST_PATH) {
        if (*c.w.status != MCQ_OK) return;
    } else if (assemble_problem(c, wveh, nullptr, nullptr) != MCQ_OK) return;
    double* red = g_sm + SM_RED;
    const int nm = B.nmax;

    const gdouble* LO = VEC(c.w, nm, V_LO);
    const gdouble* HI = VEC(c.w, nm, V_HI);
    const gdouble* F = VEC(c.w, nm, V_F);
    gdouble* X = VEC(c.w, nm, V_X);
    gdouble* G = VEC(c.w, nm, V_G);
    gdouble* T0 = VEC(c.w, nm, V_T0);
    gdouble* T1 = VEC(c.w, nm, V_T1);
    gdouble* T2 = VEC(c.w, nm, V_T2);
    gdouble* T3 = VEC(c.w, nm, V_T3);
    gdouble* Q = VEC(c.w, nm, V_Q);
    gschar* ST = c.w.state;

    if (!c.direct) {
        gdouble* Fw = VEC(c.w, nm, V_F);
        tri_apply_Et(c, VEC(c.w, nm, V_KREF), Fw);
        EB_FOR {
            EB_INDEX
            double f[EB_E];
            EB_EACH f[u] = Fw[idx[u]];
            EB_EACH if (ok[u]) Fw[idx[u]] = f[u] * MCQ_F_SCALE;
        }
        __syncthreads();
    }
    problem_scales(c);
    const bool gi_only = B.algorithm == MCQ_ALG_GI && !c.direct && (B.gi != nullptr || B.gis != nullptr);

    int ipm_iters = 0, as_iters = 0, nact_kappa = 0;
    double kkt = 0.0;
    const bool small = n <= IPB_E * MCQ_NT;
    bool warm_done = false;
    if (IN.warm && small && !gi_only) {
        const gschar* WS = (const gschar*)(IN.warm + (size_t)pb * nm);
        for (int i = tid; i < n; i += MCQ_NT)
            if (ST[i] == 0) { const signed char s = WS[i]; ST[i] = (s == 1 || s == -1) ? s : (signed char)0; }
        __syncthreads();
        const int capw = B.max_as_iter < MCQ_WARM_ROUNDS ? B.max_as_iter : MCQ_WARM_ROUNDS;
        const int sw = active_set(c, false, false, capw, 0, kappa_mem_lds(c));
        as_iters = c.out_iters;
        kkt = c.out_kkt;
        if (sw == MCQ_OK) warm_done = true;
        else {
            c.second_attempt = 2;
            for (int i = tid; i < n; i += MCQ_NT) {
                ST[i] = !(HI[i] - LO[i] > 1e-12) ? 2 : 0;
                X[i] = 0.5 * (LO[i] + HI[i]);
            }
            __syncthreads();
            gradient(c, X, nullptr, T0, G);
        }
    }
    const int as_warm = warm_done ? 0 : as_iters;
    int status = MCQ_OK;
    const long long t_ipm0 = TICK();
    if (gi_only) status = MCQ_ITER_CAP;
    else if (!warm_done) {
        status = small ? ipm_box(c, MCQ_IPM_TOL, false) : ipm(c, false);
        ipm_iters = c.out_iters;
        __syncthreads();
    }
    if (tid == 0) c.tk[4] = TICK() - t_ipm0;
    const long long t_as0 = TICK();
    if (warm_done) {
    } else if (status == MCQ_OK && small) {
        gdouble* XS = VEC(c.w, nm, V_TL);
        EB_FOR {
            EB_INDEX
            double x[EB_E];
            EB_EACH x[u] = X[idx[u]];
            EB_EACH if (ok[u]) XS[idx[u]] = x[u];
        }
        const int cap1 = B.max_as_iter < 6 ? B.max_as_iter : 6;
        status = active_set(c, false, ipm_iters >= 1 && c.last_step >= 0.9, cap1, 1, kappa_mem_lds(c));
        as_iters = c.out_iters;
        kkt = c.out_kkt;
        if (status == MCQ_ITER_CAP && B.max_as_iter > cap1) {
            c.second_attempt |= 1;
            for (int i = tid; i < n; i += MCQ_NT) X[i] = XS[i];
            __syncthreads();
            status = ipm_box(c, 1e-13, true);
            ipm_iters += c.out_iters;
            __syncthreads();
            if (status == MCQ_OK) {
                status = active_set(c, false, false, B.max_as_iter, 1, kappa_mem_lds(c));
                as_iters += c.out_iters;
                kkt = c.out_kkt;
            }
        }
    } else if (status == MCQ_OK) {
        status = active_set(c, false, ipm_iters >= 1 && c.last_step >= 0.9, B.max_as_iter, 1, kappa_mem_lds(c));
        as_iters = c.out_iters;
        kkt = c.out_kkt;
    }
    if (c.direct && status == MCQ_ITER_CAP) {
        status = active_set(c, false, false, 8 * n + 200, 0, kappa_mem_lds(c));
        as_iters += c.out_iters;
        kkt = c.out_kkt;
        if (tid == 0) c.second_attempt |= 4;
    }
    as_iters += as_warm;
    if (tid == 0) c.tk[5] = TICK() - t_as0;
    const long long t_epi0 = TICK();

    EB_FOR {
        EB_INDEX
        double x[EB_E], lo[EB_E], hi[EB_E];
        EB_EACH { const int i = idx[u]; x[u] = X[i]; lo[u] = LO[i]; hi[u] = HI[i]; }
        EB_EACH if (ok[u]) X[idx[u]] = fmin(fmax(x[u], lo[u]), hi[u]);
    }
    __syncthreads();
    double km = 0.0;
    bool dd_valid = false;
    if (!c.direct) {
        tri_apply_E(c, X, VEC(c.w, nm, V_KREF), 1.0, T0, VEC(c.w, nm, V_TL), VEC(c.w, nm, V_TU));
        dd_valid = true;
        EB_FOR {
            EB_INDEX
            double t0[EB_E];
            EB_EACH t0[u] = T0[idx[u]];
            EB_EACH if (ok[u]) km = fmax(km, fabs(t0[u]));
        }
        km = block_reduce_(km, 2, red);
    }

    if (status == MCQ_OK && B.check_kappa && !c.direct && km > kbound * (1.0 + 1e-9)) {
        dd_valid = false;
        status = ipm(c, true);
        ipm_iters += c.out_iters;
        __syncthreads();
        if (status == MCQ_OK) {
            status = active_set(c, true, false, B.max_as_iter, 1, kappa_mem_lds(c));
            as_iters += c.out_iters;
            kkt = c.out_kkt;
            nact_kappa = c.out_nk;
            if (status == MCQ_KAPPA_ACTIVE && B.kbig && B.kbig_slots > 0) {
                const int slot = claim_slot(B.slot_flags, B.kbig_slots, false);
                if (slot >= 0) {
                    status = active_set(c, true, false, B.max_as_iter, 0, kappa_mem_slot(B.kbig + (size_t)slot * MCQ_KBIG_SLOT));
                    as_iters += c.out_iters;
                    kkt = c.out_kkt;
                    nact_kappa = c.out_nk;
                    release_slot(B.slot_flags, slot);
                } else status = MCQ_KAPPA_NO_SLOT;
            }
        }
        for (int i = tid; i < n; i += MCQ_NT) X[i] = fmin(fmax(X[i], LO[i]), HI[i]);
        __syncthreads();
        tri_apply_E(c, X, VEC(c.w, nm, V_KREF), 1.0, T0);
        double k2 = 0.0;
        for (int i = tid; i < n; i += MCQ_NT) k2 = fmax(k2, fabs(T0[i]));
        km = block_reduce_(k2, 2, red);
        if (status == MCQ_OK && km > kbound * (1.0 + 1e-8)) status = MCQ_KAPPA_ACTIVE;
    } else if (status == MCQ_OK && !B.check_kappa && !c.direct && km > kbound * (1.0 + 1e-9)) {
        status = MCQ_KAPPA_ACTIVE;
    }

    int gi_iters = 0;
    if (!c.direct && (B.gi || B.gis) && gi_eligible(status, B.check_kappa)) {
        status = gi_rescue(c, B, B.check_kappa != 0, status, as_iters, nact_kappa, kkt, km, gi_iters);
        dd_valid = true;
    }
    McqOutcome r;
    r.status = status; r.ipm_iters = ipm_iters; r.as_iters = as_iters; r.nact_kappa = nact_kappa; r.gi_iters = gi_iters;
    r.kkt = kkt; r.km = km; r.dd_valid = dd_valid;
    r.t_kernel0 = t_kernel0; r.c_kernel0 = c_kernel0; r.t_epi0 = t_epi0;
    write_outputs(c, r);
}

__global__ void __launch_bounds__(MCQ_NT, 2) mcq_solve_kernel(McqBatch B)
{
    solve_body(B, mcq_set_of(B), B.pb0 + (int)blockIdx.x);
}

#define RL_KW 48
__device__ void relin_spline_c(const gdouble* RX, const gdouble* RY, int n, gdouble* CX, gdouble* CY)
{
    const double lam = sqrt(3.0) - 2.0, A = 1.0 / (4.0 + 2.0 * lam);
    for (int i = threadIdx.x; i < n; i += MCQ_NT) {
        double cx, cy;
        if (n > 2 * RL_KW) {
            cx = A * RX[i];
            cy = A * RY[i];
            double g = A;
            int ju = i, jd = i;
            for (int k = 1; k <= RL_KW; ++k) {
                g *= lam;
                ju = ju + 1 == n ? 0 : ju + 1;
                jd = jd == 0 ? n - 1 : jd - 1;
                cx += g * (RX[ju] + RX[jd]);
                cy += g * (RY[ju] + RY[jd]);
            }
        } else {
            double ln = 1.0;
            for (int k = 0; k < n; ++k) ln *= lam;
            const double sc = A / (1.0 - ln), il = 1.0 / lam;
            double pk = 1.0, qk = ln;
            cx = 0.0;
            cy = 0.0;
            int j = i;
            for (int k = 0; k < n; ++k) {
                const double g = sc * (pk + qk);
                cx += g * RX[j];
                cy += g * RY[j];
                pk *= lam;
                qk *= il;
                j = j + 1 == n ? 0 : j + 1;
            }
        }
        CX[i] = cx;
        CY[i] = cy;
    }
}

__device__ void relin_spline_rhs(const gdouble* PX, const gdouble* PY, int n, gdouble* RX, gdouble* RY)
{
    for (int i = threadIdx.x; i < n; i += MCQ_NT) {
        const int ip = i + 1 == n ? 0 : i + 1, im = i == 0 ? n - 1 : i - 1;
        RX[i] = 3.0 * ((PX[ip] - PX[i]) - (PX[i] - PX[im]));
        RY[i] = 3.0 * ((PY[ip] - PY[i]) - (PY[i] - PY[im]));
    }
}

#define RELIN_LDS 2050
__device__ __forceinline__ int relin_front(const gdouble* ref, const gdouble* nv, const gdouble* al, int n, double alpha_scale,
                                           double stepsize, gdouble* vec, size_t nm, double& total, double* lds)
{
    double* sbuf = lds;
    double& s_carry = lds[2048];
    int& s_m = *(int*)(lds + 2049);
    const int tid = threadIdx.x;
    gdouble* PX = vec + 0 * nm;   gdouble* PY = vec + 1 * nm;
    gdouble* RX = vec + 2 * nm;   gdouble* RY = vec + 3 * nm;
    gdouble* CX = vec + 4 * nm;   gdouble* CY = vec + 5 * nm;
    gdouble* LEN = vec + 6 * nm;  gdouble* CUM = vec + 7 * nm;
    gdouble* WR = vec + 8 * nm;   gdouble* WL = vec + 9 * nm;

    for (int i = tid; i < n; i += MCQ_NT) {
        const double a = alpha_scale * al[i];
        PX[i] = ref[4 * i] + a * nv[2 * i];
        PY[i] = ref[4 * i + 1] + a * nv[2 * i + 1];
        WR[i] = ref[4 * i + 2] - a;
        WL[i] = ref[4 * i + 3] + a;
    }
    __syncthreads();
    relin_spline_rhs(PX, PY, n, RX, RY);
    __syncthreads();
    relin_spline_c(RX, RY, n, CX, CY);
    __syncthreads();

    for (int i = tid; i < n; i += MCQ_NT) {
        const int ip = i + 1 == n ? 0 : i + 1;
        const double ax = PX[i], ay = PY[i], cx = CX[i], cy = CY[i];
        const double dlx = PX[ip] - ax, dly = PY[ip] - ay;
        const double bx = dlx - (2.0 * cx + CX[ip]) / 3.0, by = dly - (2.0 * cy + CY[ip]) / 3.0;
        const double dx = (CX[ip] - cx) / 3.0, dy = (CY[ip] - cy) / 3.0;
        double len = 0.0, x0 = ax, y0 = ay;
        for (int k = 1; k < 15; ++k) {
            const double t = (double)k / 14.0;
            const double x1 = ax + bx * t + cx * t * t + dx * t * t * t;
            const double y1 = ay + by * t + cy * t * t + dy * t * t * t;
            len += hypot(x1 - x0, y1 - y0);
            x0 = x1;
            y0 = y1;
        }
        LEN[i] = len;
    }
    __syncthreads();
    if (tid == 0) s_carry = 0.0;
    for (int c0 = 0; c0 < n; c0 += 2048) {
        const int cn = n - c0 < 2048 ? n - c0 : 2048;
        __syncthreads();
        for (int q = tid; q < cn; q += MCQ_NT) sbuf[q] = LEN[c0 + q];
        __syncthreads();
        if (tid == 0) {
            double acc = s_carry;
            for (int q = 0; q < cn; ++q) { acc += sbuf[q]; sbuf[q] = acc; }
            s_carry = acc;
        }
        __syncthreads();
        for (int q = tid; q < cn; q += MCQ_NT) CUM[c0 + q] = sbuf[q];
    }
    __syncthreads();
    total = s_carry;
    if (tid == 0) {
        const double cnt = ceil(total / stepsize) + 1.0;
        s_m = (cnt >= 2.0 && cnt <= 2.0e9) ? (int)cnt - 1 : -1;
    }
    __syncthreads();
    return s_m;
}

struct McqRelinIO {
    const int* n_in; const double* ref_in; const double* nv_in;
    double* ref_out; double* nv_out; int* n_out;
    double alpha_scale;
};
__device__ __forceinline__ void relin_body(const McqRelin& R, const McqRelinIO& IO, const int pb, double* lds)
{
    const int tid = threadIdx.x;
    if (R.live && R.live[pb] == 0) return;
    const size_t nm = (size_t)R.nmax;
    const int n = IO.n_in[pb];
    const gdouble* ref = (const gdouble*)(IO.ref_in + (size_t)pb * nm * 4);
    const gdouble* nv = (const gdouble*)(IO.nv_in + (size_t)pb * nm * 2);
    const gdouble* al = (const gdouble*)(R.alpha + (size_t)pb * nm);
    gdouble* refo = (gdouble*)(IO.ref_out + (size_t)pb * nm * 4);
    gdouble* nvo = (gdouble*)(IO.nv_out + (size_t)pb * nm * 2);
    gdouble* vec = (gdouble*)(R.vec + (size_t)pb * nm * MCQ_NVEC);
    gdouble* PX = vec + 0 * nm;   gdouble* PY = vec + 1 * nm;
    gdouble* CX = vec + 4 * nm;   gdouble* CY = vec + 5 * nm;
    gdouble* LEN = vec + 6 * nm;  gdouble* CUM = vec + 7 * nm;
    gdouble* WR = vec + 8 * nm;   gdouble* WL = vec + 9 * nm;
    gdouble* QX = vec + 10 * nm;  gdouble* QY = vec + 11 * nm;
    gint* n_out = (gint*)(IO.n_out + pb);
    gint* status = (gint*)(R.status + pb);
    if (n < 3) {
        if (tid == 0) { *status = MCQ_BAD_INPUT; *n_out = n; }
        return;
    }
    double total;
    const int m = relin_front(ref, nv, al, n, IO.alpha_scale, R.stepsize, vec, nm, total, lds);
    if (m < 3 || m > R.nmax) {
        if (tid == 0) { *status = MCQ_BAD_INPUT; *n_out = n; }
        return;
    }

    const double step = total / (double)m;
    for (int j = tid; j < m; j += MCQ_NT) {
        const double q = (double)j * step;
        int lo = 0, hi = n;
        while (lo < hi) {
            const int mid = (lo + hi) >> 1;
            if (CUM[mid] > q) hi = mid; else lo = mid + 1;
        }
        const int s = lo < n - 1 ? lo : n - 1;
        const int sp = s + 1 == n ? 0 : s + 1;
        const double start = s > 0 ? CUM[s - 1] : 0.0;
        const double t = (q - start) / LEN[s];
        const double ax = PX[s], ay = PY[s], cx = CX[s], cy = CY[s];
        const double bx = (PX[sp] - ax) - (2.0 * cx + CX[sp]) / 3.0, by = (PY[sp] - ay) - (2.0 * cy + CY[sp]) / 3.0;
        const double dx = (CX[sp] - cx) / 3.0, dy = (CY[sp] - cy) / 3.0;
        QX[j] = ax + t * (bx + t * (cx + t * dx));
        QY[j] = ay + t * (by + t * (cy + t * dy));
        refo[4 * j + 2] = WR[s] + (WR[sp] - WR[s]) * t;
        refo[4 * j + 3] = WL[s] + (WL[sp] - WL[s]) * t;
        if (R.state_out) {
            const signed char so = ((const gschar*)(R.state_in + (size_t)pb * nm))[t > 0.5 ? sp : s];
            ((gschar*)(R.state_out + (size_t)pb * nm))[j] = (so == 1 || so == -1) ? so : (signed char)0;
        }
    }
    __syncthreads();
    for (int j = tid; j < m; j += MCQ_NT) {
        refo[4 * j] = QX[j];
        refo[4 * j + 1] = QY[j];
    }
    relin_spline_rhs(QX, QY, m, PX, PY);
    __syncthreads();
    relin_spline_c(PX, PY, m, CX, CY);
    __syncthreads();
    for (int j = tid; j < m; j += MCQ_NT) {
        const int jp = j + 1 == m ? 0 : j + 1;
        const double bx = (QX[jp] - QX[j]) - (2.0 * CX[j] + CX[jp]) / 3.0;
        const double by = (QY[jp] - QY[j]) - (2.0 * CY[j] + CY[jp]) / 3.0;
        const double nrm = sqrt(by * by + bx * bx);
        nvo[2 * j] = by / nrm;
        nvo[2 * j + 1] = -bx / nrm;
    }
    if (tid == 0) { *status = MCQ_OK; *n_out = m; }
}

__global__ void __launch_bounds__(MCQ_NT) mcq_relinearise_kernel(McqRelin R)
{
    __shared__ double lds[RELIN_LDS];
    McqRelinIO io;
    io.n_in = R.n_in; io.ref_in = R.ref_in; io.nv_in = R.nv_in; io.ref_out = R.ref_out; io.nv_out = R.nv_out; io.n_out = R.n_out;
    io.alpha_scale = R.alpha_scale;
    relin_body(R, io, (int)blockIdx.x, lds);
}

__device__ __forceinline__ void iqp_step_track(const McqIqpStep& S, int k, int phase, int round, int cur, const int* n_ring, int* n_next, bool count)
{
    if (phase == 0) {
        if (S.live[k] == 0) return;
        const int st = S.status[k];
        const double ce = S.curv[k];
        S.final_n[k] = n_ring[k];
        S.final_buf[k] = cur;
        S.final_curv[k] = ce;
        S.final_status[k] = st;
        S.final_rounds[k] = round;
        if (S.curv_trace && round <= MCQ_IQP_TRACE) S.curv_trace[(size_t)k * MCQ_IQP_TRACE + round - 1] = ce;
        const bool stop = st != MCQ_OK || (round >= S.iters_min && ce <= S.curv_allowed);
        if (stop) S.live[k] = 0;
        else if (count) atomicAdd(S.live_count, 1);
    } else {
        if (S.live[k] != 0 && S.relin_status[k] != MCQ_OK) {
            S.live[k] = 0;
            S.final_status[k] = MCQ_RING_OVERFLOW;
            if (count) atomicAdd(S.live_count, -1);
        }
        if (S.live[k] == 0) n_next[k] = 0;
    }
}

__global__ void __launch_bounds__(256) mcq_iqp_step_kernel(McqIqpStep S)
{
    const int k = (int)blockIdx.x * 256 + (int)threadIdx.x;
    if (k >= S.batch) return;
    iqp_step_track(S, k, S.phase, S.round, S.cur, S.n_ring, S.n_next, true);
}

__global__ void __launch_bounds__(MCQ_NT, 2) mcq_iqp_rounds_kernel(McqIqpRounds F)
{
    const int pb = (int)blockIdx.x;
    for (int it = 1; it <= F.rounds; ++it) {
        const int cur = (it - 1) & 1;
        if (F.S.live[pb] == 0) {
            if (threadIdx.x == 0) { F.n_set[0][pb] = 0; F.n_set[1][pb] = 0; }
            break;
        }
        McqSet in;
        in.n_list = F.n_set[cur];
        in.ref = F.ref_set[cur];
        in.nv = F.nv_set[cur];
        in.sc = it == 1 ? F.sc : nullptr;
        in.warm = it > 1 ? F.warm : nullptr;
        solve_body(F.B, in, pb);
        __syncthreads();
        if (threadIdx.x == 0) iqp_step_track(F.S, pb, 0, it, cur, F.n_set[cur], F.n_set[1 - cur], it == F.rounds);
        __syncthreads();
        McqRelinIO io;
        io.n_in = F.n_set[cur]; io.ref_in = F.ref_set[cur]; io.nv_in = F.nv_set[cur];
        io.ref_out = F.ref_set[1 - cur]; io.nv_out = F.nv_set[1 - cur]; io.n_out = F.n_set[1 - cur];
        io.alpha_scale = it < F.S.iters_min ? (double)it / (double)F.S.iters_min : 1.0;
        relin_body(F.R, io, pb, g_sm);
        __syncthreads();
        if (threadIdx.x == 0) iqp_step_track(F.S, pb, 1, it, cur, F.n_set[cur], F.n_set[1 - cur], it == F.rounds);
        __syncthreads();
    }
}

__device__ __forceinline__ double vp_interp(double x, const gdouble* tab, int cnt, int stride, int col)
{
    if (x <= tab[0]) return tab[col];
    if (x >= tab[(size_t)(cnt - 1) * stride]) return tab[(size_t)(cnt - 1) * stride + col];
    int k = 1;
    while (k < cnt - 1 && tab[(size_t)k * stride] <= x) ++k;
    const double x0 = tab[(size_t)(k - 1) * stride], x1 = tab[(size_t)k * stride];
    const double y0 = tab[(size_t)(k - 1) * stride + col], y1 = tab[(size_t)k * stride + col];
    return y0 + (y1 - y0) * (x - x0) / (x1 - x0);
}

__device__ __forceinline__ double vp_ax_from_limits(double ax_t, double ay_t, double v, double rad, const gdouble* axm, int nam, bool accel,
                                                    double e, double drag_over_m)
{
    const double ay_used = v * v / rad;
    const double radicand = 1.0 - pow(ay_used / ay_t, e);
    const double ax_tires = radicand > 0.0 ? ax_t * pow(radicand, 1.0 / e) : 0.0;
    const double ax_drag = -v * v * drag_over_m;
    if (accel) return fmin(ax_tires, vp_interp(v, axm, nam, 2, 1)) + ax_drag;
    return ax_tires - ax_drag;
}

__device__ __forceinline__ double vp_ax_possible(double v, double rad, double mu, const gdouble* ggv, int ng, const gdouble* axm, int nam,
                                                 bool accel, double e, double drag_over_m)
{
    const double ax_t = fabs(mu * vp_interp(v, ggv, ng, 3, 1)), ay_t = mu * vp_interp(v, ggv, ng, 3, 2);
// ... 1559 lines not shown
```

### global_racetrajectory_optimization_amd/csrc/mcq_tri.inc

```
#define TRI_W 64
#define TRI_LD 2488
#define TRI_MAXN MCQ_TRI_MAXN
#define TRI_PAD(m) ((m) + ((m) >> 3))
#define TRI_H (TRI_W + 8)
#define TRI_PE(e) ((e) + ((e) >> 3))
#define TRI_X(i) TRI_PE((i) + TRI_H)
__device__ __forceinline__ int tri_ring(int e, int n)
{
    int i = e - TRI_H;
    if (n >= TRI_H) return i < 0 ? i + n : i >= n ? i - n : i;
    i %= n;
    return i < 0 ? i + n : i;
}
#ifndef TRI_UNR
#define TRI_UNR 8
#endif
static_assert(TRI_MAXN == 8 * MCQ_NT && TRI_PE(TRI_MAXN + 2 * TRI_H - 1) < TRI_LD && TRI_W % 8 == 0, "padded LDS rows of the tridiagonal solves, halo included");
static_assert(3 * TRI_LD <= OVL_SIZE, "right-hand side, 1 / delta and u of the tridiagonal solves must fit the LDS overlay");


__device__ void tri_prepare(const LCtx& c)
{
    const int n = c.d.n, tid = threadIdx.x;
    const gdouble* SC = VEC(c.w, c.nm, V_SC);
    gdouble* IDL = VEC(c.w, c.nm, V_IDL);
    gdouble* TUC = VEC(c.w, c.nm, V_TUC);
    __syncthreads();
    if (c.chain) {
        for (int m0 = 8 * tid; m0 < n; m0 += 8 * MCQ_NT) {
            const int mb = m0 >= TRI_W ? m0 - TRI_W : 0;
            double idl = 0.0, uprev = 0.0;
            for (int m = mb; m < m0 + 8 && m < n; ++m) {
                const double sp = m > 0 ? SC[m - 1] : 1.0, sm = SC[m];
                const double d = (m == 0 || m == n - 1) ? 2.0 : 2.0 * sp * sp + 2.0 * sp;
                const double u = m == n - 1 ? 0.0 : sp * sm * sm;
                const double delta = d - uprev * idl;
                idl = 1.0 / delta;
                uprev = u;
                if (m >= m0) { IDL[m] = idl; TUC[m] = u; }
            }
        }
        __syncthreads();
        return;
    }
    for (int base = 0; base < n; base += 8 * MCQ_NT) {
        const int m0 = base + 8 * tid;
        if (m0 < n) {
            int m = m0 - TRI_W;
            m %= n;
            if (m < 0) m += n;
            int mp = m > 0 ? m - 1 : n - 1;
            double sp = SC[mp];
            double idl = 0.0, uprev = 0.0;
            for (int k = -TRI_W; k < 8; ++k) {
                const double sm = SC[m];
                const double d = 2.0 * sp * sp + 2.0 * sp, u = sp * sm * sm;
                const double delta = d - uprev * idl;
                idl = 1.0 / delta;
                uprev = u;
                if (k >= 0 && m0 + k < n) { IDL[m0 + k] = idl; TUC[m0 + k] = u; }
                sp = sm;
                m = m + 1 < n ? m + 1 : 0;
            }
        }
    }
    __syncthreads();
}

struct TriLds {
    double* ry;
    double* idl;
    double* tu;
};
__device__ __forceinline__ TriLds tri_lds()
{
    TriLds t;
    t.ry = g_sm + SM_OVL;
    t.idl = g_sm + SM_OVL + TRI_LD;
    t.tu = g_sm + SM_OVL + 2 * TRI_LD;
    return t;
}
__device__ __forceinline__ void tri_put(double* arr, int n, int i, double v, bool chain)
{
    const int e = i + TRI_H;
    if (chain) {
        arr[TRI_PE(e)] = v;
    } else if (n >= TRI_H) {
        arr[TRI_PE(e)] = v;
        if (e >= n) arr[TRI_PE(e - n)] = v;
        if (i < TRI_H) arr[TRI_PE(e + n)] = v;
    } else {
        for (int q = e % n; q < n + 2 * TRI_H; q += n) arr[TRI_PE(q)] = v;
    }
}
__device__ __forceinline__ int tri_win(int m0, int k, int n)
{
    const int j = m0 + k;
    return j < 0 ? n - 1 : j < n ? j : 0;
}
__device__ __forceinline__ void tri_stage_factors(const LCtx& c, const TriLds& L)
{
    const int n = c.d.n, m0 = 8 * threadIdx.x;
    const gdouble* IDL = VEC(c.w, c.nm, V_IDL);
    const gdouble* TUC = VEC(c.w, c.nm, V_TUC);
    const bool chain = c.chain != 0;
    if (chain) {
        for (int q = threadIdx.x; q < 2 * TRI_H; q += MCQ_NT) {
            const int e = q < TRI_H ? q : n + q;
            L.ry[TRI_PE(e)] = 0.0;
            L.idl[TRI_PE(e)] = 0.0;
            L.tu[TRI_PE(e)] = 0.0;
        }
    }
    if (m0 >= n) return;
    double a[8], b[8];
#pragma unroll
    for (int k = 0; k < 8; ++k) { a[k] = IDL[tri_win(m0, k, n)]; b[k] = TUC[tri_win(m0, k, n)]; }
#pragma unroll
    for (int k = 0; k < 8; ++k)
        if (m0 + k < n) { tri_put(L.idl, n, m0 + k, a[k], chain); tri_put(L.tu, n, m0 + k, b[k], chain); }
}

template <bool TRANS>
__device__ __forceinline__ void tri_solve_chunk(const TriLds& L, int n, double (&own)[8], bool chain)
{
    const int tid = threadIdx.x, m0 = 8 * tid;
    const bool valid = m0 < n;
    const int t9 = valid ? 9 * tid : 0;
    double y = 0.0;
#pragma unroll 1
    for (int a = 1; a <= TRI_W / 8; ++a) {
        const int q = t9 + 9 * a;
#pragma unroll
        for (int kk = 0; kk < 8; ++kk) {
            const int sp = kk == 0 ? q - 2 : q + kk - 1;
            const double f = TRANS ? L.tu[sp] * L.idl[sp] : L.idl[sp];
            y = fma(-f, y, L.ry[q + kk]);
        }
    }
    const int qo = t9 + 9 * (TRI_W / 8 + 1);
#pragma unroll
    for (int kk = 0; kk < 8; ++kk) {
        const int sp = kk == 0 ? qo - 2 : qo + kk - 1;
        const double f = TRANS ? L.tu[sp] * L.idl[sp] : L.idl[sp];
        y = fma(-f, y, L.ry[qo + kk]);
        own[kk] = y;
    }
    __syncthreads();
    if (valid)
        for (int k = 0; k < 8; ++k)
            if (m0 + k < n)
                for (int e = m0 + k + TRI_H; e < (chain ? m0 + k + TRI_H + 1 : n + 2 * TRI_H); e += n) L.ry[TRI_PE(e)] = own[k];
    __syncthreads();
    double x = 0.0;
#pragma unroll 1
    for (int a = TRI_W / 8; a >= 1; --a) {
        const int q = qo + 9 * a;
#pragma unroll
        for (int kk = 7; kk >= 0; --kk) {
            const double yk = L.ry[q + kk];
            x = TRANS ? (yk - x) * L.idl[q + kk] : (yk - L.tu[q + kk] * x) * L.idl[q + kk];
        }
    }
#pragma unroll
    for (int kk = 7; kk >= 0; --kk) {
        const double yk = (valid && m0 + kk < n) ? own[kk] : L.ry[qo + kk];
        x = TRANS ? (yk - x) * L.idl[qo + kk] : (yk - L.tu[qo + kk] * x) * L.idl[qo + kk];
        own[kk] = x;
    }
}

template <bool TRANS>
__device__ void tri_solve_long(const LCtx& c, const gdouble* R, gdouble* Y, gdouble* X)
{
    const int n = c.d.n, tid = threadIdx.x;
    const gdouble* IDL = VEC(c.w, c.nm, V_IDL);
    const gdouble* TU = VEC(c.w, c.nm, V_TUC);
    __syncthreads();
    for (int base = 0; base < n; base += 8 * MCQ_NT) {
        const int m0 = base + 8 * tid;
        if (m0 >= n) continue;
        int m = (m0 - TRI_W) % n;
        if (m < 0) m += n;
        int mp = m > 0 ? m - 1 : n - 1;
        double y = 0.0;
#pragma unroll 8
        for (int k = -TRI_W; k < 8; ++k) {
            const double f = TRANS ? TU[mp] * IDL[mp] : IDL[mp];
            y = fma(-f, y, R[m]);
            if (k >= 0 && m0 + k < n) Y[m0 + k] = y;
            mp = m;
            m = m + 1 < n ? m + 1 : 0;
        }
    }
    __syncthreads();
    for (int base = 0; base < n; base += 8 * MCQ_NT) {
        const int m0 = base + 8 * tid;
        if (m0 >= n) continue;
        int mm = (m0 + 7 + TRI_W) % n;
        double x = 0.0;
#pragma unroll 8
        for (int k = 7 + TRI_W; k >= 0; --k) {
            const double yk = Y[mm];
            x = TRANS ? (yk - x) * IDL[mm] : (yk - TU[mm] * x) * IDL[mm];
            if (k < 8 && m0 + k < n) X[m0 + k] = x;
            mm = mm > 0 ? mm - 1 : n - 1;
        }
    }
    __syncthreads();
}

__device__ __noinline__ void tri_solve_T(const LCtx& c, const gdouble* rhs, gdouble* out)
{
    const int n = c.d.n, tid = threadIdx.x;
    if (n > TRI_MAXN) { tri_solve_long<false>(c, rhs, K_TS(c, 1), out); return; }
    const TriLds L = tri_lds();
    __syncthreads();
    tri_stage_factors(c, L);
    const int m0 = 8 * tid;
    double own[8];
    if (m0 < n) {
#pragma unroll
        for (int k = 0; k < 8; ++k) own[k] = rhs[tri_win(m0, k, n)];
#pragma unroll
        for (int k = 0; k < 8; ++k)
            if (m0 + k < n) tri_put(L.ry, n, m0 + k, own[k], c.chain != 0);
    }
    __syncthreads();
    tri_solve_chunk<false>(L, n, own, c.chain != 0);
    if (m0 < n) {
#pragma unroll
        for (int k = 0; k < 8; ++k)
            if (m0 + k < n) out[m0 + k] = own[k];
    }
    __syncthreads();
}

__device__ __noinline__ void tri_apply_E_lds(const LCtx& c, const gdouble* src, const gdouble* add, double addc, gdouble* dst,
                                             gdouble* d1, gdouble* d2)
{
    const int n = c.d.n, tid = threadIdx.x;
    const gdouble* SC = VEC(c.w, c.nm, V_SC);
    const gdouble* NX = VEC(c.w, c.nm, V_NX);
    const gdouble* NY = VEC(c.w, c.nm, V_NY);
    const gdouble* XP = VEC(c.w, c.nm, V_XP);
    const gdouble* YP = VEC(c.w, c.nm, V_YP);
    const gdouble* CP = VEC(c.w, c.nm, V_CP);
    const TriLds L = tri_lds();
    const bool chain = c.chain != 0;
    __syncthreads();
    tri_stage_factors(c, L);
    double c1[8], c2[8];
    const int m0 = 8 * tid;
    const bool mine = m0 < n;
    double sv[10], sc[8];
    if (mine) {
#pragma unroll
        for (int k = -1; k <= 8; ++k) sv[k + 1] = src[tri_win(m0, k, n)];
#pragma unroll
        for (int k = 0; k < 8; ++k) sc[k] = SC[tri_win(m0, k - 1, n)];
    }
#pragma unroll
    for (int pass = 0; pass < 2; ++pass) {
        const gdouble* NV = pass == 0 ? NX : NY;
        __syncthreads();
        if (mine) {
            double q[10];
#pragma unroll
            for (int k = -1; k <= 8; ++k) q[k + 1] = NV[tri_win(m0, k, n)] * sv[k + 1];
#pragma unroll
            for (int k = 0; k < 8; ++k)
                if (m0 + k < n) tri_put(L.ry, n, m0 + k, 3.0 * q[k] - 3.0 * (sc[k] + 1.0) * q[k + 1] + 3.0 * sc[k] * q[k + 2], chain);
            if (chain) {
                if (m0 == 0) L.ry[TRI_X(0)] = 3.0 * (q[2] - q[1]);
#pragma unroll
                for (int k = 0; k < 8; ++k)
                    if (m0 + k == n - 1) L.ry[TRI_X(n - 1)] = 3.0 * (q[k] - q[k + 1]);
            }
        }
        __syncthreads();
        if (pass == 0) tri_solve_chunk<false>(L, n, c1, chain);
        else tri_solve_chunk<false>(L, n, c2, chain);
    }
    if (mine) {
        double cp[8], xp[8], yp[8], ad[8];
#pragma unroll
        for (int k = 0; k < 8; ++k) {
            const int m = tri_win(m0, k, n);
            cp[k] = CP[m]; xp[k] = XP[m]; yp[k] = YP[m];
            ad[k] = add ? add[m] : 0.0;
        }
#pragma unroll
        for (int k = 0; k < 8; ++k) {
            const int m = m0 + k;
            if (m < n) {
                double v = (-2.0 * cp[k] * yp[k]) * c1[k] + (2.0 * cp[k] * xp[k]) * c2[k];
                if (add) v += addc * ad[k];
                dst[m] = v;
                if (d1) { d1[m] = 2.0 * c1[k]; d2[m] = 2.0 * c2[k]; }
            }
        }
    }
    __syncthreads();
}
__device__ __noinline__ void tri_apply_E_long(const LCtx& c, const gdouble* src, const gdouble* add, double addc, gdouble* dst,
                                              gdouble* d1, gdouble* d2)
{
    const int n = c.d.n, tid = threadIdx.x;
    const gdouble* SC = VEC(c.w, c.nm, V_SC);
    const gdouble* XP = VEC(c.w, c.nm, V_XP);
    const gdouble* YP = VEC(c.w, c.nm, V_YP);
    const gdouble* CP = VEC(c.w, c.nm, V_CP);
    gdouble* R = K_TS(c, 0);
    gdouble* Y = K_TS(c, 1);
    gdouble* C = K_TS(c, 2);
    for (int pass = 0; pass < 2; ++pass) {
        const gdouble* NV = VEC(c.w, c.nm, pass == 0 ? V_NX : V_NY);
        __syncthreads();
        for (int i = tid; i < n; i += MCQ_NT) {
            const int im = i > 0 ? i - 1 : n - 1, ip = i + 1 < n ? i + 1 : 0;
            const double s1 = SC[im];
            R[i] = 3.0 * (NV[im] * src[im]) - 3.0 * (s1 + 1.0) * (NV[i] * src[i]) + 3.0 * s1 * (NV[ip] * src[ip]);
        }
        tri_solve_long<false>(c, R, Y, C);
        for (int i = tid; i < n; i += MCQ_NT) {
            const double cp = CP[i], ci = C[i];
            if (pass == 0) {
                dst[i] = (-2.0 * cp * YP[i]) * ci + (add ? addc * add[i] : 0.0);
                if (d1) d1[i] = 2.0 * ci;
            } else {
                dst[i] += (2.0 * cp * XP[i]) * ci;
                if (d2) d2[i] = 2.0 * ci;
            }
        }
    }
    __syncthreads();
}
__device__ __forceinline__ void tri_apply_E(const LCtx& c, const gdouble* src, const gdouble* add, double addc, gdouble* dst,
                                            gdouble* d1 = nullptr, gdouble* d2 = nullptr)
{
    if (c.d.n <= TRI_MAXN) tri_apply_E_lds(c, src, add, addc, dst, d1, d2);
    else tri_apply_E_long(c, src, add, addc, dst, d1, d2);
}

__device__ __noinline__ void tri_apply_Et_lds(const LCtx& c, const gdouble* src, gdouble* dst)
{
    const int n = c.d.n, tid = threadIdx.x;
    const gdouble* SC = VEC(c.w, c.nm, V_SC);
    const gdouble* NX = VEC(c.w, c.nm, V_NX);
    const gdouble* NY = VEC(c.w, c.nm, V_NY);
    const gdouble* XP = VEC(c.w, c.nm, V_XP);
    const gdouble* YP = VEC(c.w, c.nm, V_YP);
    const gdouble* CP = VEC(c.w, c.nm, V_CP);
    const TriLds L = tri_lds();
    const bool chain = c.chain != 0;
    __syncthreads();
    tri_stage_factors(c, L);
    double acc[8], ce0 = 0.0, cen = 0.0;
#pragma unroll
    for (int k = 0; k < 8; ++k) acc[k] = 0.0;
    const int m0 = 8 * tid;
    const bool mine = m0 < n;
    double wy[8], wx[8], sc[9];
    if (mine) {
#pragma unroll
        for (int k = 0; k < 8; ++k) {
            const int m = tri_win(m0, k, n);
            const double cp = CP[m], sm = src[m];
            wy[k] = (-2.0 * cp * YP[m]) * sm;
            wx[k] = (2.0 * cp * XP[m]) * sm;
        }
        sc[0] = SC[m0 >= 2 ? m0 - 2 : (m0 - 2 + n) % n];
#pragma unroll
        for (int k = 1; k < 9; ++k) sc[k] = SC[tri_win(m0, k - 2, n)];
    }
#pragma unroll
    for (int pass = 0; pass < 2; ++pass) {
        const gdouble* NV = pass == 0 ? NX : NY;
        __syncthreads();
        if (mine) {
#pragma unroll
            for (int k = 0; k < 8; ++k)
                if (m0 + k < n) tri_put(L.ry, n, m0 + k, pass == 0 ? wy[k] : wx[k], chain);
        }
        __syncthreads();
        double u[8];
        tri_solve_chunk<true>(L, n, u, chain);
        __syncthreads();
        double nv[8];
        if (mine) {
#pragma unroll
            for (int k = 0; k < 8; ++k) {
                nv[k] = NV[tri_win(m0, k, n)];
                if (m0 + k < n) L.ry[TRI_X(m0 + k)] = u[k];
            }
        }
        __syncthreads();
        if (mine) {
            const double ub = L.ry[TRI_X(m0 > 0 ? m0 - 1 : n - 1)];
            const int ml = m0 + 7 < n ? m0 + 7 : n - 1;
            const double ua = L.ry[TRI_X(ml + 1 < n ? ml + 1 : 0)];
#pragma unroll
            for (int k = 0; k < 8; ++k) {
                const int m = m0 + k;
                if (m < n) {
                    const double um = k > 0 ? u[k - 1] : ub;
                    const double up = m == ml ? ua : u[k < 7 ? k + 1 : 7];
                    const double rt = 3.0 * sc[k] * um - 3.0 * (sc[k + 1] + 1.0) * u[k] + 3.0 * up;
                    acc[k] += nv[k] * rt;
                }
            }
            if (chain && tid == 0) {
                ce0 += NV[0] * (3.0 * (L.ry[TRI_X(1)] - L.ry[TRI_X(0)]));
                cen += NV[n - 1] * (3.0 * (SC[n - 3] * L.ry[TRI_X(n - 2)] - L.ry[TRI_X(n - 1)]));
            }
        }
    }
    if (mine) {
#pragma unroll
        for (int k = 0; k < 8; ++k)
            if (m0 + k < n) dst[m0 + k] = acc[k];
    }
    __syncthreads();
    if (chain) {
        if (tid == 0) { dst[0] = ce0; dst[n - 1] = cen; }
        __syncthreads();
    }
}
__device__ __noinline__ void tri_apply_Et_long(const LCtx& c, const gdouble* src, gdouble* dst)
{
    const int n = c.d.n, tid = threadIdx.x;
    const gdouble* SC = VEC(c.w, c.nm, V_SC);
    const gdouble* XP = VEC(c.w, c.nm, V_XP);
    const gdouble* YP = VEC(c.w, c.nm, V_YP);
    const gdouble* CP = VEC(c.w, c.nm, V_CP);
    gdouble* R = K_TS(c, 0);
    gdouble* Y = K_TS(c, 1);
    gdouble* U = K_TS(c, 2);
    for (int pass = 0; pass < 2; ++pass) {
        const gdouble* NV = VEC(c.w, c.nm, pass == 0 ? V_NX : V_NY);
        __syncthreads();
        for (int i = tid; i < n; i += MCQ_NT) {
            const double cp = CP[i];
            R[i] = (pass == 0 ? -2.0 * cp * YP[i] : 2.0 * cp * XP[i]) * src[i];
        }
        tri_solve_long<true>(c, R, Y, U);
        for (int m = tid; m < n; m += MCQ_NT) {
            const int mm = m > 0 ? m - 1 : n - 1, m2 = mm > 0 ? mm - 1 : n - 1, mp = m + 1 < n ? m + 1 : 0;
            const double rt = 3.0 * SC[m2] * U[mm] - 3.0 * (SC[mm] + 1.0) * U[m] + 3.0 * U[mp];
            dst[m] = pass == 0 ? NV[m] * rt : dst[m] + NV[m] * rt;
        }
    }
    __syncthreads();
}
__device__ __forceinline__ void tri_apply_Et(const LCtx& c, const gdouble* src, gdouble* dst)
{
    if (c.d.n <= TRI_MAXN) tri_apply_Et_lds(c, src, dst);
    else tri_apply_Et_long(c, src, dst);
}

#define V_SPD V_XP
#define V_SPU V_YP
#define V_SPZ V_IDL
#define V_SPA V_XPP
#define V_SPB V_YPP
#define V_SPC V_TUC
#define SP_PA 0
#define SP_PP (4 * MCQ_NT)
static_assert(7 * MCQ_NT <= SPK, "separator system of the scalar tridiagonal solves must fit the persistent LDS region");

template <typename P, bool PAD>
__device__ __forceinline__ bool sp_chain_solve(P d, P o, P r, int n)
{
#define SPX(i) (PAD ? TRI_PAD(i) : (i))
    const int tid = threadIdx.x;
    const int m = (n + MCQ_NT - 1) / MCQ_NT, nb = (n + m - 1) / m;
    double* pa = g_sm + SM_S + SP_PA;
    double* pb = pa + MCQ_NT;
    double* pc = pb + MCQ_NT;
    double* pd = pc + MCQ_NT;
    double* pp = g_sm + SM_S + SP_PP;
    double* pq = pp + MCQ_NT;
    double* pw = pq + MCQ_NT;
    const bool has = tid < nb;
    const int s = tid * m;
    const int e = has ? ((s + m < n ? s + m : n) - 1) : 0;
    const int mi = has ? e - s : 0;
    bool bad = false;
    double p = 0.0, q = 0.0, w = 0.0, p1 = 0.0, q1 = 0.0, w1 = 0.0;
    if (mi > 0) {
        const double cl = tid > 0 ? o[SPX(s - 1)] : 0.0;
        double u = d[SPX(s)], rr = r[SPX(s)], ff = cl;
        for (int k = s + 1; k < e; ++k) {
            const double ok = o[SPX(k - 1)];
            bad |= !(u > 0.0);
            const double mlt = ok * kkt_rcp(u);
            u = fma(-mlt, ok, d[SPX(k)]);
            rr = fma(-mlt, rr, r[SPX(k)]);
            ff = -mlt * ff;
        }
        bad |= !(u > 0.0);
        double iu = kkt_rcp(u);
        p = rr * iu; q = ff * iu; w = o[SPX(e - 1)] * iu;
        double u2 = d[SPX(e - 1)], r2 = r[SPX(e - 1)], gg = o[SPX(e - 1)];
        for (int k = e - 2; k >= s; --k) {
            const double ok = o[SPX(k)];
            bad |= !(u2 > 0.0);
            const double mlt = ok * kkt_rcp(u2);
            u2 = fma(-mlt, ok, d[SPX(k)]);
            r2 = fma(-mlt, r2, r[SPX(k)]);
            gg = -mlt * gg;
        }
        bad |= !(u2 > 0.0);
        iu = kkt_rcp(u2);
        p1 = r2 * iu; q1 = cl * iu; w1 = gg * iu;
    }
    pp[tid] = p1; pq[tid] = q1; pw[tid] = w1;
    __syncthreads();
    double ra = 0.0, rb = 1.0, rc = 0.0, rd = 0.0;
    if (has) {
        const double ae = e > 0 ? o[SPX(e - 1)] : 0.0;
        const double ce = e < n - 1 ? o[SPX(e)] : 0.0;
        const int tn = tid + 1;
        const int min_ = tn < nb ? ((tn * m + m < n ? tn * m + m : n) - 1 - tn * m) : 0;
        rb = d[SPX(e)];
        rd = r[SPX(e)];
        if (mi > 0) { ra = -ae * q; rb = fma(-ae, w, rb); rd = fma(-ae, p, rd); }
        else ra = ae;
        if (min_ > 0) { rc = -ce * pw[tn]; rb = fma(-ce, pq[tn], rb); rd = fma(-ce, pp[tn], rd); }
        else rc = ce;
    }
    pa[tid] = ra; pb[tid] = rb; pc[tid] = rc; pd[tid] = rd;
    __syncthreads();
    for (int st = 1; st < nb; st <<= 1) {
        const int il = tid - st, ir = tid + st;
        double al = 0.0, bl = 1.0, cl_ = 0.0, dl = 0.0, ar = 0.0, br = 1.0, cr = 0.0, dr = 0.0;
// ... 101 lines not shown
```

Baseline: 102,700.

## Trim block reductions, fold scalings, and fuse epilogue passes in the min-curv solver

This bundles several independent trims, each behind its own macro and enabled by default. Block reductions alternate between two LDS banks to drop a barrier, and sibling reductions are merged into one pass. The tridiagonal prepare stages the scale factors in LDS, the factor of 2 and the F scaling are folded into existing loops, and a cold IPM start skips one setup pass. The epilogue fuses clamping, the alpha write and the active count. A bitwise-comparison build variant with everything disabled is added, and the risk is subtle barrier or ordering bugs from the bank reuse.

```diff
diff --git a/__graft_entry__.py b/__graft_entry__.py
--- a/__graft_entry__.py
+++ b/__graft_entry__.py
@@ -36,6 +36,8 @@
 
 VARIANTS = {"ulp": (["-DMCQ_PERTURB_ULP=1"], {}), "ipra": ([], {"IPRA": "1"}), "nocontract": (["-ffp-contract=off"], {}),
             "nof32": (["-DMCQ_IPM_F32=0"], {})}
+BITWISE_VARIANTS = {"trim0": (["-DMCQ_RED_BANKS=0", "-DMCQ_RED_MERGE=0", "-DMCQ_TRI_PREP_STAGE=0", "-DMCQ_TRI_FOLD_TWICE=0", "-DMCQ_PRO_FOLD_F=0",
+                               "-DMCQ_IPB_COLD_SKIP=0", "-DMCQ_IPB_XS_FLUSH=0", "-DMCQ_EPI_FUSE=0"], {})}
 
 
 def variant_path(name):
@@ -45,7 +47,7 @@
 def build_variants() -> None:
     os.makedirs(os.path.dirname(variant_path("x")), exist_ok=True)
     procs = []
-    for name, (flags, extra) in VARIANTS.items():
+    for name, (flags, extra) in {**VARIANTS, **BITWISE_VARIANTS}.items():
         env = dict(os.environ)
         env.setdefault("HIPCC", "/opt/rocm/bin/hipcc")
         env.pop("ASM_OUT", None)
diff --git a/global_racetrajectory_optimization_amd/csrc/mcq_kernels.hip b/global_racetrajectory_optimization_amd/csrc/mcq_kernels.hip
--- a/global_racetrajectory_optimization_amd/csrc/mcq_kernels.hip
+++ b/global_racetrajectory_optimization_amd/csrc/mcq_kernels.hip
@@ -104,6 +104,114 @@
     }
     a = ra;
     b = rb;
+}
+
+#ifndef MCQ_RED_BANKS
+#define MCQ_RED_BANKS 1
+#endif
+#ifndef MCQ_RED_MERGE
+#define MCQ_RED_MERGE 1
+#endif
+#define RED_BANK_LD 16
+static_assert(2 * RED_BANK_LD <= 32 && 3 * MCQ_NW <= RED_BANK_LD, "two banks of three values below the shortest path's flag (SM_RED + 32)");
+__device__ __forceinline__ double red_op_(double a, double b, int op) { return op == 0 ? a + b : (op == 1 ? fmin(a, b) : fmax(a, b)); }
+__device__ __forceinline__ double block_reduce_b_(double v, int op, double* red, int bank)
+{
+#if MCQ_RED_BANKS
+    const int lane = threadIdx.x & 63, wv = threadIdx.x >> 6;
+    double* rb = red + bank * RED_BANK_LD;
+    v = op == 0 ? wave_sum(v) : (op == 1 ? wave_min(v) : wave_max(v));
+    if (lane == 0) rb[wv] = v;
+    __syncthreads();
+    double r = rb[0];
+    for (int k = 1; k < MCQ_NW; ++k) r = red_op_(r, rb[k], op);
+    return r;
+#else
+    (void)bank;
+    return block_reduce_(v, op, red);
+#endif
+}
+__device__ __forceinline__ void block_reduce2b_(double& a, int opa, double& b, int opb, double* red, int bank)
+{
+#if MCQ_RED_BANKS
+    const int lane = threadIdx.x & 63, wv = threadIdx.x >> 6;
+    double* rb = red + bank * RED_BANK_LD;
+    for (int m = 32; m >= 1; m >>= 1) {
+        const double oa = __shfl_xor(a, m), ob = __shfl_xor(b, m);
+        a = red_op_(a, oa, opa);
+        b = red_op_(b, ob, opb);
+    }
+    if (lane == 0) { rb[wv] = a; rb[MCQ_NW + wv] = b; }
+    __syncthreads();
+    double ra = rb[0], rbb = rb[MCQ_NW];
+    for (int k = 1; k < MCQ_NW; ++k) {
+        ra = red_op_(ra, rb[k], opa);
+        rbb = red_op_(rbb, rb[MCQ_NW + k], opb);
+    }
+    a = ra;
+    b = rbb;
+#else
+    (void)bank;
+    block_reduce2_(a, opa, b, opb, red);
+#endif
+}
+__device__ __forceinline__ void block_reduce2m_(double& a, int opa, double& b, int opb, double* red, int bank)
+{
+#if MCQ_RED_MERGE
+    block_reduce2b_(a, opa, b, opb, red, bank);
+#else
+    a = block_reduce_b_(a, opa, red, bank);
+    b = block_reduce_b_(b, opb, red, bank ^ 1);
+#endif
+}
+__device__ __forceinline__ void block_reduce3b_(double& a, int opa, double& b, int opb, double& c3, int opc, double* red, int bank)
+{
+#if MCQ_RED_MERGE && MCQ_RED_BANKS
+    const int lane = threadIdx.x & 63, wv = threadIdx.x >> 6;
+    double* rb = red + bank * RED_BANK_LD;
+    for (int m = 32; m >= 1; m >>= 1) {
+        const double oa = __shfl_xor(a, m), ob = __shfl_xor(b, m), oc = __shfl_xor(c3, m);
+        a = red_op_(a, oa, opa);
+        b = red_op_(b, ob, opb);
+        c3 = red_op_(c3, oc, opc);
+    }
+    if (lane == 0) { rb[wv] = a; rb[MCQ_NW + wv] = b; rb[2 * MCQ_NW + wv] = c3; }
+    __syncthreads();
+    double ra = rb[0], rbb = rb[MCQ_NW], rc = rb[2 * MCQ_NW];
+    for (int k = 1; k < MCQ_NW; ++k) {
+        ra = red_op_(ra, rb[k], opa);
+        rbb = red_op_(rbb, rb[MCQ_NW + k], opb);
+        rc = red_op_(rc, rb[2 * MCQ_NW + k], opc);
+    }
+    a = ra;
+    b = rbb;
+    c3 = rc;
+#elif MCQ_RED_MERGE
+    const int lane = threadIdx.x & 63, wv = threadIdx.x >> 6;
+    (void)bank;
+    for (int m = 32; m >= 1; m >>= 1) {
+        const double oa = __shfl_xor(a, m), ob = __shfl_xor(b, m), oc = __shfl_xor(c3, m);
+        a = red_op_(a, oa, opa);
+        b = red_op_(b, ob, opb);
+        c3 = red_op_(c3, oc, opc);
+    }
+    __syncthreads();
+    if (lane == 0) { red[wv] = a; red[MCQ_NW + wv] = b; red[2 * MCQ_NW + wv] = c3; }
+    __syncthreads();
+    double ra = red[0], rbb = red[MCQ_NW], rc = red[2 * MCQ_NW];
+    for (int k = 1; k < MCQ_NW; ++k) {
+        ra = red_op_(ra, red[k], opa);
+        rbb = red_op_(rbb, red[MCQ_NW + k], opb);
+        rc = red_op_(rc, red[2 * MCQ_NW + k], opc);
+    }
+    a = ra;
+    b = rbb;
+    c3 = rc;
+#else
+    a = block_reduce_b_(a, opa, red, bank);
+    b = block_reduce_b_(b, opb, red, bank ^ 1);
+    c3 = block_reduce_b_(c3, opc, red, bank);
+#endif
 }
 
 struct McqSet {
@@ -267,8 +375,7 @@
             S[i] = s;
         }
     }
-    flag_bad = block_reduce_(flag_bad, 2, red);
-    flag_inf = block_reduce_(flag_inf, 2, red);
+    block_reduce2m_(flag_bad, 2, flag_inf, 2, red, 0);
     const int st = flag_bad > 0.0 ? MCQ_BAD_INPUT : (flag_inf > 0.0 ? MCQ_INFEASIBLE : MCQ_OK);
     if (tid == 0) {
         *w.status = st;
@@ -319,15 +426,17 @@
         RX[n - 1] = 3.0 * (hex - (w.ref[4 * (n - 1)] - w.ref[4 * (n - 2)]));
         RY[n - 1] = 3.0 * (hey - (w.ref[4 * (n - 1) + 1] - w.ref[4 * (n - 2) + 1]));
     }
-    tri_solve_T(c, RX, XPP);
-    tri_solve_T(c, RY, YPP);
-    EB_FOR {
-        EB_INDEX
-        double a[EB_E], b[EB_E];
-        EB_EACH { a[u] = XPP[idx[u]]; b[u] = YPP[idx[u]]; }
-        EB_EACH if (ok[u]) { XPP[idx[u]] = a[u] * 2.0; YPP[idx[u]] = b[u] * 2.0; }
-    }
-    __syncthreads();
+    tri_solve_T(c, RX, XPP, true);
+    tri_solve_T(c, RY, YPP, true);
+    if (!MCQ_TRI_FOLD_TWICE || n > TRI_MAXN) {
+        EB_FOR {
+            EB_INDEX
+            double a[EB_E], b[EB_E];
+            EB_EACH { a[u] = XPP[idx[u]]; b[u] = YPP[idx[u]]; }
+            EB_EACH if (ok[u]) { XPP[idx[u]] = a[u] * 2.0; YPP[idx[u]] = b[u] * 2.0; }
+        }
+        __syncthreads();
+    }
 
     EB_FOR {
         EB_INDEX
@@ -819,6 +928,15 @@
 #ifndef MCQ_IPB_FOLD_P1
 #define MCQ_IPB_FOLD_P1 1
 #endif
+#ifndef MCQ_IPB_COLD_SKIP
+#define MCQ_IPB_COLD_SKIP MCQ_IPB_DEFER
+#endif
+#ifndef MCQ_IPB_XS_FLUSH
+#define MCQ_IPB_XS_FLUSH MCQ_IPB_DEFER
+#endif
+#if (MCQ_IPB_COLD_SKIP || MCQ_IPB_XS_FLUSH) && !MCQ_IPB_DEFER
+#error "MCQ_IPB_COLD_SKIP and MCQ_IPB_XS_FLUSH need MCQ_IPB_DEFER"
+#endif
 __device__ __noinline__ int ipm_box(const LCtx& c, double tol, bool resume)
 {
 #define IPB_SETUP                                                                                                      \
@@ -874,7 +992,7 @@
     const double zscale = c.zscale;
     const double IPM_TOL = tol;
     c.out_iters = 0;
-    {
+    if (!(MCQ_IPB_COLD_SKIP && !resume)) {
     IPB_SETUP
 #if MCQ_ENTRY_BATCH
     double lo[IPB_E], hi[IPB_E];
@@ -900,18 +1018,37 @@
     }
 #undef IPB_LO
 #undef IPB_HI
-    }
-    __syncthreads();
+    __syncthreads();
+    }
     if (resume) gradient(c, VEC(c.w, c.nm, V_X), nullptr, VEC(c.w, c.nm, V_T0), VEC(c.w, c.nm, V_G));
     const double npairs = 2.0 * c.nfree;
     const bool any_fixed = c.nfree < (double)c.d.n;
-    if (!(npairs > 0.0)) return MCQ_OK;
+    if (!(npairs > 0.0)) {
+#if MCQ_IPB_COLD_SKIP || MCQ_IPB_XS_FLUSH
+        if (!resume) {
+            IPB_SETUP
+#pragma unroll
+            for (int u = 0; u < IPB_E; ++u) {
+                if (!ok[u]) continue;
+                const int i = idx[u];
+                if (MCQ_IPB_COLD_SKIP) { ZL[i] = 0.0; ZU[i] = 0.0; }
+                if (MCQ_IPB_XS_FLUSH) VEC(c.w, nm, V_TL)[i] = X[i];
+            }
+        }
+#endif
+        return MCQ_OK;
+    }
 #if MCQ_IPB_RESIDENT
     double rx[IPB_E], rl[IPB_E], ru[IPB_E], rg[IPB_E];
     {
         IPB_SETUP
 #pragma unroll
-        for (int u = 0; u < IPB_E; ++u) { const int i = idx[u]; rx[u] = X[i]; rl[u] = ZL[i]; ru[u] = ZU[i]; rg[u] = G[i]; }
+        for (int u = 0; u < IPB_E; ++u) {
+            const int i = idx[u];
+            rx[u] = X[i]; rg[u] = G[i];
+            if (MCQ_IPB_COLD_SKIP && !resume) { rl[u] = ST[i] == 2 ? 0.0 : zscale; ru[u] = rl[u]; }
+            else { rl[u] = ZL[i]; ru[u] = ZU[i]; }
+        }
     }
 #define IPB_RELOAD_G { _Pragma("unroll") for (int u = 0; u < IPB_E; ++u) rg[u] = G[tid + u * MCQ_NT < n ? tid + u * MCQ_NT : 0]; }
 #else
@@ -983,7 +1120,7 @@
                     RHS[i] = -g[u];
                 }
             }
-            block_reduce2_(mu, 0, rdm, 2, red);
+            block_reduce2b_(mu, 0, rdm, 2, red, 0);
             mu /= npairs;
             }
             const bool conv = mu < IPM_TOL * zscale * c.wmean && rdm < IPM_TOL * zscale;
@@ -1057,7 +1194,7 @@
                 if (dzla < 0.0) ad = fmin(ad, -zl[u] / dzla);
                 if (dzua < 0.0) ad = fmin(ad, -zu[u] / dzua);
             }
-            block_reduce2_(ap, 1, ad, 1, red);
+            block_reduce2b_(ap, 1, ad, 1, red, 0);
             double mua = 0.0;
 #pragma unroll
             for (int u = 0; u < IPB_E; ++u) {
@@ -1066,7 +1203,7 @@
                 const double dzua = -zu[u] + zu[u] * dxa[u] / su[u];
                 mua += (sl[u] + ap * dxa[u]) * (zl[u] + ad * dzla) + (su[u] - ap * dxa[u]) * (zu[u] + ad * dzua);
             }
-            mua = block_reduce_(mua, 0, red) / npairs;
+            mua = block_reduce_b_(mua, 0, red, 1) / npairs;
             const double ratio = mua / mu;
             smu = ratio * ratio * ratio * mu;
 #pragma unroll
@@ -1114,7 +1251,7 @@
                 if (dzl < 0.0) amax = fmin(amax, -zl[u] / dzl);
                 if (dzu < 0.0) amax = fmin(amax, -zu[u] / dzu);
             }
-            amax = block_reduce_(amax, 1, red);
+            amax = block_reduce_b_(amax, 1, red, 0);
             const double a = fmin(1.0, gm * amax);
             c.last_step = a;
 #if MCQ_IPB_DEFER
@@ -1165,7 +1302,7 @@
 #endif
             }
 #if MCQ_IPB_FOLD_P1
-            block_reduce2_(mu_n, 0, rdm_n, 2, red);
+            block_reduce2b_(mu_n, 0, rdm_n, 2, red, 1);
             mu_fold = mu_n / npairs;
             rdm_fold = rdm_n;
             folded = true;
@@ -1193,6 +1330,7 @@
             if (!ok[u]) continue;
             const int i = idx[u];
             X[i] = rx[u]; ZL[i] = rl[u]; ZU[i] = ru[u]; G[i] = rg[u];
+            if (MCQ_IPB_XS_FLUSH && !resume) VEC(c.w, nm, V_TL)[i] = rx[u];
             const unsigned t = (tapia >> (2 * u)) & 3u;
             if (t != 0) IND[i] = (double)((int)t - 2);
         }
@@ -1532,9 +1670,8 @@
                 if (vk != 0) { nv += 1.0; imax = fmax(imax, (double)(n + i)); }
             }
         }
-        nv = block_reduce_(nv, 0, red);
-        imax = block_reduce_(imax, 2, red);
-        c.out_kkt = block_reduce_(kk, 2, red);
+        block_reduce3b_(nv, 0, imax, 2, kk, 2, red, 0);
+        c.out_kkt = kk;
         const int nvi = (int)nv;
         if (nvi == 0) {
             for (int r = 0; r < c.refine_steps; ++r) {
@@ -1570,7 +1707,7 @@
                     EB_EACH { const int i = idx[u]; st[u] = ST[i]; x[u] = X[i]; rh[u] = RHS[i]; }
                     EB_EACH if (ok[u] && st[u] == 0) { X[idx[u]] = x[u] + rh[u]; dm = fmax(dm, fabs(rh[u])); }
                 }
-                dm = block_reduce_(dm, 2, red);
+                dm = block_reduce_b_(dm, 2, red, 0);
                 gradient(c, X, nk > 0 ? Q : nullptr, T0, G);
                 if (nk > 0) tri_apply_E(c, X, KR, 1.0, T2);
                 c.refine_rounds = r + 1;
@@ -1584,7 +1721,7 @@
                 EB_EACH { const int i = idx[u]; st[u] = ST[i]; g[u] = G[i]; }
                 EB_EACH if (ok[u] && st[u] == 0) k2 = fmax(k2, fabs(g[u]));
             }
-            c.out_kkt = block_reduce_(k2, 2, red);
+            c.out_kkt = block_reduce_b_(k2, 2, red, 1);
             return MCQ_OK;
         }
         bool full;
@@ -1646,16 +1783,20 @@
 #else
 #define MCQ_FN_PROLOGUE __device__ __forceinline__
 #endif
-MCQ_FN_PROLOGUE void problem_scales(const LCtx& c)
+#ifndef MCQ_PRO_FOLD_F
+#define MCQ_PRO_FOLD_F 1
+#endif
+MCQ_FN_PROLOGUE void problem_scales(const LCtx& c, bool scale_f)
 {
     const int tid = threadIdx.x, n = c.d.n, nm = c.nm;
     double* red = g_sm + SM_RED;
     const gdouble* LO = VEC(c.w, nm, V_LO);
     const gdouble* HI = VEC(c.w, nm, V_HI);
-    const gdouble* F = VEC(c.w, nm, V_F);
+    gdouble* F = VEC(c.w, nm, V_F);
     gdouble* X = VEC(c.w, nm, V_X);
     gdouble* G = VEC(c.w, nm, V_G);
     gschar* ST = c.w.state;
+    (void)scale_f;
     double wsum = 0.0, nfree_d = 0.0, fmaxl = 0.0;
     EB_FOR {
         EB_INDEX
@@ -1669,11 +1810,14 @@
             ST[i] = fixed ? 2 : 0;
             X[i] = 0.5 * (lo[u] + hi[u]);
             if (!fixed) { wsum += wdt; nfree_d += 1.0; }
+#if MCQ_PRO_FOLD_F
+            if (scale_f) { f[u] = f[u] * MCQ_F_SCALE; F[i] = f[u]; }
+#endif
             fmaxl = fmax(fmaxl, fabs(f[u]));
         }
     }
-    wsum = block_reduce_(wsum, 0, red);
-    const double nfree_s = block_reduce_(nfree_d, 0, red), fscale_s = block_reduce_(fmaxl, 2, red);
+    block_reduce3b_(wsum, 0, nfree_d, 0, fmaxl, 2, red, 0);
+    const double nfree_s = nfree_d, fscale_s = fmaxl;
     gradient(c, X, nullptr, VEC(c.w, nm, V_T0), G);
     double gm = 0.0;
     EB_FOR {
@@ -1683,7 +1827,7 @@
         EB_EACH { const int i = idx[u]; st[u] = ST[i]; g[u] = G[i]; }
         EB_EACH if (ok[u] && st[u] == 0) gm = fmax(gm, fabs(g[u]));
     }
-    double zscale_s = block_reduce_(gm, 2, red);
+    double zscale_s = block_reduce_b_(gm, 2, red, 0);
     if (!(zscale_s > 0.0)) zscale_s = fscale_s > 0.0 ? fscale_s : 1.0;
     if (tid == 0) {
         g_ctx.nfree = nfree_s;
@@ -1694,10 +1838,20 @@
     __syncthreads();
 }
 
+#ifndef MCQ_EPI_FUSE
+#define MCQ_EPI_FUSE 1
+#endif
+#ifndef MCQ_EPI_POSTCHECK_BATCH
+#define MCQ_EPI_POSTCHECK_BATCH 4
+#endif
+#define EPQ_E (MCQ_ENTRY_BATCH ? MCQ_EPI_POSTCHECK_BATCH : 1)
+#define RED_BANK_BEHIND_2M(bank) (MCQ_RED_MERGE ? (bank) ^ 1 : (bank))
 struct McqOutcome {
     int status, ipm_iters, as_iters, nact_kappa, gi_iters;
     double kkt, km;
     bool dd_valid;
+    bool fused;
+    double nact;
     long long t_kernel0, c_kernel0, t_epi0;
 };
 MCQ_FN_PROLOGUE void write_outputs(const LCtx& c, const McqOutcome& r)
@@ -1711,7 +1865,9 @@
     gdouble* T3 = VEC(c.w, nm, V_T3);
     gdouble* Q = VEC(c.w, nm, V_Q);
     const gschar* ST = c.w.state;
-    double nact = 0.0;
+    double nact = r.nact;
+    if (!r.fused) {
+    nact = 0.0;
     EB_FOR {
         EB_INDEX
         signed char st[EB_E];
@@ -1723,11 +1879,62 @@
             if (st[u] == -1 || st[u] == 1) nact += 1.0;
         }
     }
-    nact = block_reduce_(nact, 0, red);
+    nact = block_reduce_b_(nact, 0, red, 1);
+    }
     const gdouble* XP = VEC(c.w, nm, V_XP);
     const gdouble* YP = VEC(c.w, nm, V_YP);
     const gdouble* XPP = VEC(c.w, nm, V_XPP);
     const gdouble* YPP = VEC(c.w, nm, V_YPP);
+#if MCQ_EPI_FUSE
+    const gdouble* DD1 = r.dd_valid ? VEC(c.w, nm, V_TL) : T0;
+    const gdouble* DD2 = r.dd_valid ? VEC(c.w, nm, V_TU) : T3;
+    if (!c.direct) {
+        if (!r.fused) {
+            EB_FOR {
+                EB_INDEX
+                double nx[EB_E], ny[EB_E], x[EB_E];
+                EB_EACH { const int i = idx[u]; nx[u] = VEC(c.w, nm, V_NX)[i]; ny[u] = VEC(c.w, nm, V_NY)[i]; x[u] = X[i]; }
+                EB_EACH if (ok[u]) { T1[idx[u]] = nx[u] * x[u]; T2[idx[u]] = ny[u] * x[u]; }
+            }
+            __syncthreads();
+        }
+        if (!r.dd_valid) tri_apply_E(c, X, nullptr, 0.0, Q, T0, T3);
+    }
+    double em = 0.0;
+    for (int eb0_ = tid; eb0_ < (c.direct ? 0 : n); eb0_ += EPQ_E * MCQ_NT) {
+        int idx[EPQ_E], idp[EPQ_E];
+        bool ok[EPQ_E];
+        double s_[EPQ_E], xp_[EPQ_E], yp_[EPQ_E], xq_[EPQ_E], yq_[EPQ_E], t1[EPQ_E], t1p[EPQ_E], t2[EPQ_E], t2p[EPQ_E], d1[EPQ_E], d1p[EPQ_E], d2[EPQ_E], d2p[EPQ_E];
+#pragma unroll
+        for (int u = 0; u < EPQ_E; ++u) {
+            ok[u] = eb0_ + u * MCQ_NT < n;
+            idx[u] = ok[u] ? eb0_ + u * MCQ_NT : eb0_;
+            idp[u] = cyc(idx[u] + 1, n);
+        }
+#pragma unroll
+        for (int u = 0; u < EPQ_E; ++u) {
+            const int i = idx[u], ip = idp[u];
+            s_[u] = VEC(c.w, nm, V_SC)[i]; xp_[u] = XP[i]; yp_[u] = YP[i]; xq_[u] = XPP[i]; yq_[u] = YPP[i];
+            t1[u] = T1[i]; t1p[u] = T1[ip]; t2[u] = T2[i]; t2p[u] = T2[ip];
+            d1[u] = DD1[i]; d1p[u] = DD1[ip]; d2[u] = DD2[i]; d2p[u] = DD2[ip];
+        }
+#pragma unroll
+        for (int u = 0; u < EPQ_E; ++u) {
+            if (!ok[u]) continue;
+            const int i = idx[u];
+            const double s2 = s_[u] * s_[u];
+            double xpt = xp_[u] + (t1p[u] - t1[u]) - (d1[u] + 0.5 * s2 * d1p[u]) / 3.0;
+            double ypt = yp_[u] + (t2p[u] - t2[u]) - (d2[u] + 0.5 * s2 * d2p[u]) / 3.0;
+            if (c.chain && i == n - 1) { xpt = xp_[u]; ypt = yp_[u]; }
+            const double xpp = xq_[u] + d1[u], ypp = yq_[u] + d2[u];
+            const double xp = xp_[u], yp = yp_[u];
+            const double k0 = (xp * ypp - yp * xpp) / pow(xp * xp + yp * yp, 1.5);
+            const double k1 = (xpt * ypp - ypt * xpp) / pow(xpt * xpt + ypt * ypt, 1.5);
+            em = fmax(em, fabs(k1 - k0));
+        }
+    }
+    em = block_reduce_b_(em, 2, red, (r.fused && !c.direct) ? RED_BANK_BEHIND_2M(0) : 0);
+#else
     if (!c.direct) {
         EB_FOR {
             EB_INDEX
@@ -1764,7 +1971,8 @@
         const double k1 = (xpt * ypp - ypt * xpp) / pow(xpt * xpt + ypt * ypt, 1.5);
         em = fmax(em, fabs(k1 - k0));
     }
-    em = block_reduce_(em, 2, red);
+    em = block_reduce_b_(em, 2, red, 0);
+#endif
     if (tid == 0) {
         *c.w.curv_err = em;
         *c.w.status = r.status;
@@ -1826,6 +2034,7 @@
     if (!c.direct) {
         gdouble* Fw = VEC(c.w, nm, V_F);
         tri_apply_Et(c, VEC(c.w, nm, V_KREF), Fw);
+#if !MCQ_PRO_FOLD_F
         EB_FOR {
             EB_INDEX
             double f[EB_E];
@@ -1833,8 +2042,9 @@
             EB_EACH if (ok[u]) Fw[idx[u]] = f[u] * MCQ_F_SCALE;
         }
         __syncthreads();
-    }
-    problem_scales(c);
+#endif
+    }
+    problem_scales(c, !c.direct);
     const bool gi_only = B.algorithm == MCQ_ALG_GI && !c.direct && (B.gi != nullptr || B.gis != nullptr);
 
     int ipm_iters = 0, as_iters = 0, nact_kappa = 0;
@@ -1875,12 +2085,14 @@
     if (warm_done) {
     } else if (status == MCQ_OK && small) {
         gdouble* XS = VEC(c.w, nm, V_TL);
+#if !MCQ_IPB_XS_FLUSH
         EB_FOR {
             EB_INDEX
             double x[EB_E];
             EB_EACH x[u] = X[idx[u]];
             EB_EACH if (ok[u]) XS[idx[u]] = x[u];
         }
+#endif
         const int cap1 = B.max_as_iter < 6 ? B.max_as_iter : 6;
         status = active_set(c, false, ipm_iters >= 1 && c.last_step >= 0.9, cap1, 1, kappa_mem_lds(c));
         as_iters = c.out_iters;
@@ -1913,15 +2125,46 @@
     if (tid == 0) c.tk[5] = TICK() - t_as0;
     const long long t_epi0 = TICK();
 
+    bool fused = false;
+    double nact = 0.0;
+#if MCQ_EPI_FUSE
+    fused = true;
+    {
+        const bool with_n = !c.direct;
+        const gdouble* NX = VEC(c.w, nm, V_NX);
+        const gdouble* NY = VEC(c.w, nm, V_NY);
+        EB_FOR {
+            EB_INDEX
+            signed char st[EB_E];
+            double x[EB_E], lo[EB_E], hi[EB_E], nx[EB_E], ny[EB_E];
+            EB_EACH {
+                const int i = idx[u];
+                st[u] = ST[i]; x[u] = X[i]; lo[u] = LO[i]; hi[u] = HI[i];
+                nx[u] = with_n ? NX[i] : 0.0; ny[u] = with_n ? NY[i] : 0.0;
+            }
+            EB_EACH {
+                if (!ok[u]) continue;
+                const int i = idx[u];
+                const double xc = fmin(fmax(x[u], lo[u]), hi[u]);
+                X[i] = xc;
+                c.w.alpha[i] = xc;
+                if (st[u] == -1 || st[u] == 1) nact += 1.0;
+                if (with_n) { T1[i] = nx[u] * xc; T2[i] = ny[u] * xc; }
+            }
+        }
+    }
+#else
     EB_FOR {
         EB_INDEX
         double x[EB_E], lo[EB_E], hi[EB_E];
         EB_EACH { const int i = idx[u]; x[u] = X[i]; lo[u] = LO[i]; hi[u] = HI[i]; }
         EB_EACH if (ok[u]) X[idx[u]] = fmin(fmax(x[u], lo[u]), hi[u]);
     }
+#endif
     __syncthreads();
     double km = 0.0;
     bool dd_valid = false;
+    bool k_over = false;
     if (!c.direct) {
         tri_apply_E(c, X, VEC(c.w, nm, V_KREF), 1.0, T0, VEC(c.w, nm, V_TL), VEC(c.w, nm, V_TU));
         dd_valid = true;
@@ -1931,11 +2174,19 @@
             EB_EACH t0[u] = T0[idx[u]];
             EB_EACH if (ok[u]) km = fmax(km, fabs(t0[u]));
         }
-        km = block_reduce_(km, 2, red);
-    }
-
-    if (status == MCQ_OK && B.check_kappa && !c.direct && km > kbound * (1.0 + 1e-9)) {
+#if MCQ_EPI_FUSE
+        block_reduce2m_(km, 2, nact, 0, red, 0);
+        k_over = km > kbound * (1.0 + 1e-9);
+    } else nact = block_reduce_b_(nact, 0, red, 1);
+#else
+        km = block_reduce_b_(km, 2, red, 0);
+        k_over = km > kbound * (1.0 + 1e-9);
+    }
+#endif
+
+    if (status == MCQ_OK && B.check_kappa && !c.direct && k_over) {
         dd_valid = false;
+        fused = false;
         status = ipm(c, true);
         ipm_iters += c.out_iters;
         __syncthreads();
@@ -1962,7 +2213,7 @@
         for (int i = tid; i < n; i += MCQ_NT) k2 = fmax(k2, fabs(T0[i]));
         km = block_reduce_(k2, 2, red);
         if (status == MCQ_OK && km > kbound * (1.0 + 1e-8)) status = MCQ_KAPPA_ACTIVE;
-    } else if (status == MCQ_OK && !B.check_kappa && !c.direct && km > kbound * (1.0 + 1e-9)) {
+    } else if (status == MCQ_OK && !B.check_kappa && !c.direct && k_over) {
         status = MCQ_KAPPA_ACTIVE;
     }
 
@@ -1970,10 +2221,11 @@
     if (!c.direct && (B.gi || B.gis) && gi_eligible(status, B.check_kappa)) {
         status = gi_rescue(c, B, B.check_kappa != 0, status, as_iters, nact_kappa, kkt, km, gi_iters);
         dd_valid = true;
+        fused = false;
     }
     McqOutcome r;
     r.status = status; r.ipm_iters = ipm_iters; r.as_iters = as_iters; r.nact_kappa = nact_kappa; r.gi_iters = gi_iters;
-    r.kkt = kkt; r.km = km; r.dd_valid = dd_valid;
+    r.kkt = kkt; r.km = km; r.dd_valid = dd_valid; r.fused = fused; r.nact = nact;
     r.t_kernel0 = t_kernel0; r.c_kernel0 = c_kernel0; r.t_epi0 = t_epi0;
     write_outputs(c, r);
 }
diff --git a/global_racetrajectory_optimization_amd/csrc/mcq_tri.inc b/global_racetrajectory_optimization_amd/csrc/mcq_tri.inc
--- a/global_racetrajectory_optimization_amd/csrc/mcq_tri.inc
+++ b/global_racetrajectory_optimization_amd/csrc/mcq_tri.inc
@@ -19,6 +19,11 @@
 static_assert(3 * TRI_LD <= OVL_SIZE, "right-hand side, 1 / delta and u of the tridiagonal solves must fit the LDS overlay");
 
 
+#ifndef MCQ_TRI_PREP_STAGE
+#define MCQ_TRI_PREP_STAGE 1
+#endif
+__device__ __forceinline__ void tri_put(double* arr, int n, int i, double v, bool chain);
+__device__ __forceinline__ int tri_win(int m0, int k, int n);
 __device__ void tri_prepare(const LCtx& c)
 {
     const int n = c.d.n, tid = threadIdx.x;
@@ -26,6 +31,67 @@
     gdouble* IDL = VEC(c.w, c.nm, V_IDL);
     gdouble* TUC = VEC(c.w, c.nm, V_TUC);
     __syncthreads();
+#if MCQ_TRI_PREP_STAGE
+    if (n <= TRI_MAXN) {
+        double* S = g_sm + SM_OVL;
+        const int m0 = 8 * tid;
+        const bool chain = c.chain != 0;
+        if (m0 < n) {
+            double a[8];
+#pragma unroll
+            for (int k = 0; k < 8; ++k) a[k] = SC[tri_win(m0, k, n)];
+#pragma unroll
+            for (int k = 0; k < 8; ++k)
+                if (m0 + k < n) tri_put(S, n, m0 + k, a[k], chain);
+        }
+        __syncthreads();
+        if (chain) {
+            if (m0 < n) {
+                const int mb = m0 >= TRI_W ? m0 - TRI_W : 0;
+                double idl = 0.0, uprev = 0.0;
+                for (int m = mb; m < m0 + 8 && m < n; ++m) {
+                    const double sp = m > 0 ? S[TRI_X(m - 1)] : 1.0, sm = S[TRI_X(m)];
+                    const double d = (m == 0 || m == n - 1) ? 2.0 : 2.0 * sp * sp + 2.0 * sp;
+                    const double u = m == n - 1 ? 0.0 : sp * sm * sm;
+                    const double delta = d - uprev * idl;
+                    idl = 1.0 / delta;
+                    uprev = u;
+                    if (m >= m0) { IDL[m] = idl; TUC[m] = u; }
+                }
+            }
+        } else if (m0 < n) {
+            const int t9 = 9 * tid;
+            double sp = S[t9 + 7];
+            double idl = 0.0, uprev = 0.0;
+#pragma unroll 1
+            for (int a = 1; a <= TRI_W / 8; ++a) {
+                const int q = t9 + 9 * a;
+#pragma unroll
+                for (int kk = 0; kk < 8; ++kk) {
+                    const double sm = S[q + kk];
+                    const double d = 2.0 * sp * sp + 2.0 * sp, u = sp * sm * sm;
+                    const double delta = d - uprev * idl;
+                    idl = 1.0 / delta;
+                    uprev = u;
+                    sp = sm;
+                }
+            }
+            const int qo = t9 + 9 * (TRI_W / 8 + 1);
+#pragma unroll
+            for (int kk = 0; kk < 8; ++kk) {
+                const double sm = S[qo + kk];
+                const double d = 2.0 * sp * sp + 2.0 * sp, u = sp * sm * sm;
+                const double delta = d - uprev * idl;
+                idl = 1.0 / delta;
+                uprev = u;
+                if (m0 + kk < n) { IDL[m0 + kk] = idl; TUC[m0 + kk] = u; }
+                sp = sm;
+            }
+        }
+        __syncthreads();
+        return;
+    }
+#endif
     if (c.chain) {
         for (int m0 = 8 * tid; m0 < n; m0 += 8 * MCQ_NT) {
             const int mb = m0 >= TRI_W ? m0 - TRI_W : 0;
@@ -210,9 +276,13 @@
     __syncthreads();
 }
 
-__device__ __noinline__ void tri_solve_T(const LCtx& c, const gdouble* rhs, gdouble* out)
+#ifndef MCQ_TRI_FOLD_TWICE
+#define MCQ_TRI_FOLD_TWICE 1
+#endif
+__device__ __noinline__ void tri_solve_T(const LCtx& c, const gdouble* rhs, gdouble* out, bool twice)
 {
     const int n = c.d.n, tid = threadIdx.x;
+    (void)twice;
     if (n > TRI_MAXN) { tri_solve_long<false>(c, rhs, K_TS(c, 1), out); return; }
     const TriLds L = tri_lds();
     __syncthreads();
@@ -231,7 +301,11 @@
     if (m0 < n) {
 #pragma unroll
         for (int k = 0; k < 8; ++k)
+#if MCQ_TRI_FOLD_TWICE
+            if (m0 + k < n) out[m0 + k] = twice ? own[k] * 2.0 : own[k];
+#else
             if (m0 + k < n) out[m0 + k] = own[k];
+#endif
     }
     __syncthreads();
 }
```

After: 103,600, median of 6. Within noise of the previous version (+0.9%).
